# qitianwu/SGFormer

Hardware: AMD Instinct MI355X
Metric: SGFormer fwd+bwd nodes/sec on ogbn-products full-graph (higher is better)
Workload: dtype bf16

## Files before the change

### include/sgf.h

```cpp
#ifndef SGF_H_
#define SGF_H_

#include <stddef.h>
#include <stdint.h>

#ifdef __cplusplus
extern "C" {
#endif

#define SGF_VERSION 661

#define SGF_F32 0
#define SGF_BF16 1
#define SGF_F32_BF16X3 2

#define SGF_OK 0
#define SGF_E_INVALID (-1)
#define SGF_E_WORKSPACE (-2)
#define SGF_E_HIP (-3)
#define SGF_E_UNSUPPORTED (-4)

int sgf_version(void);
const char* sgf_last_error(void);
int sgf_reload_env(void);

size_t sgf_csr_workspace_bytes(int64_t nnz, int64_t n);
int sgf_csr_build(const int64_t* edge_index, int64_t nnz, int64_t n, int64_t* rowptr,
                  int32_t* colind, float* val, int32_t* deg, void* workspace,
                  size_t workspace_bytes, void* stream);

int sgf_csr_transpose(const int64_t* edge_index, int64_t nnz, int64_t n, const int32_t* deg,
                      const int64_t* rowptr, const int32_t* colind, int64_t* t_rowptr,
                      int32_t* t_colind, float* t_val, int32_t* is_symmetric, void* workspace,
                      size_t workspace_bytes, void* stream);

size_t sgf_subgraph_workspace_bytes(int64_t nnz, int64_t n);
int sgf_subgraph_plan(const int64_t* edge_index, int64_t nnz, int64_t n, const int64_t* subset,
                      int64_t m, int32_t* relabel, int64_t* total, void* workspace,
                      size_t workspace_bytes, void* stream);
int sgf_subgraph_emit(const int64_t* edge_index, int64_t nnz, int64_t n, const int32_t* relabel,
                      int32_t relabel_nodes, int64_t total, int64_t* out, int64_t* out_eid,
                      void* workspace, size_t workspace_bytes, void* stream);

size_t sgf_subgraph_csr_plan_workspace_bytes(int64_t m);
size_t sgf_subgraph_csr_emit_workspace_bytes(int64_t m, int64_t total);
int sgf_subgraph_csr_plan(const int64_t* rowptr, const int32_t* colind, int64_t n, const int64_t* subset, int64_t m,
                          int32_t* local_of, int64_t* rowptr_b, int32_t* deg_b, int64_t* total, void* workspace,
                          size_t workspace_bytes, void* stream);
int sgf_subgraph_csr_emit(const int64_t* rowptr, const int32_t* colind, int64_t n, const int64_t* subset, int64_t m,
                          int32_t* local_of, const int64_t* rowptr_b, const int32_t* deg_b, int64_t total, int32_t* colind_b,
                          float* val_b, int64_t* edge_index_b, void* workspace, size_t workspace_bytes, void* stream);

size_t sgf_graph_prologue_workspace_bytes(int64_t m, int64_t n);
int sgf_graph_prologue_plan(const int64_t* edge_index, int64_t m, int64_t n, int32_t to_undirected,
                            int32_t remove_self_loops, int32_t add_self_loops, int64_t* total,
                            void* workspace, size_t workspace_bytes, void* stream);
int sgf_graph_prologue_emit(int64_t m, int64_t n, int32_t to_undirected, int32_t add_self_loops,
                            int64_t total, int64_t* out, void* workspace, size_t workspace_bytes,
                            void* stream);

int sgf_spmm(const int64_t* rowptr, const int32_t* colind, const float* val, const void* x,
             int64_t ldx, int64_t n_cols, void* y, int64_t ldy, int64_t n_rows, int32_t d,
             int32_t dtype, void* stream);

int32_t sgf_spmm_segment_len(void);
size_t sgf_spmm_split_workspace_bytes(int64_t long_segments, int32_t d);
int sgf_spmm_split(const int64_t* rowptr, const int32_t* colind, const float* val, const void* x,
                   int64_t ldx, int64_t n_cols, void* y, int64_t ldy, int64_t n_rows, int32_t d, int32_t dtype,
                   int64_t long_len, int64_t long_segments, void* workspace, size_t workspace_bytes,
                   void* stream);

int sgf_spmm_stream(const int64_t* rowptr, const int32_t* colind, const float* val, const void* x,
                    int64_t ldx, int64_t n_cols, void* y, int64_t ldy, int64_t n_rows, int32_t d, int32_t dtype,
                    int64_t long_len, int64_t long_segments, void* workspace, size_t workspace_bytes,
                    void* stream);

size_t sgf_reorder_workspace_bytes(int64_t nnz, int64_t n);
int sgf_reorder(const int64_t* edge_index, int64_t nnz, int64_t n, int32_t iters1, int32_t iters2,
                int32_t* perm, int32_t* inv, int32_t* community, void* workspace, size_t workspace_bytes,
                void* stream);
size_t sgf_spmm_plan_workspace_bytes(int64_t nnz, int64_t n, int32_t rows_per_block);
int sgf_spmm_plan(const int64_t* rowptr, const int32_t* colind, const float* val, int64_t n, int64_t nnz,
                  int32_t rows_per_block, int32_t lds_rows, int64_t long_len, int32_t* ecode, float* eval,
                  int32_t* nlds, int32_t* sh_ptr, int32_t* sh_cols, int64_t* stats, void* workspace,
                  size_t workspace_bytes, void* stream);
int32_t sgf_spmm_lds_rows_len(int32_t dtype);
int sgf_spmm_blocked(const int64_t* rowptr, const int32_t* ecode, const float* eval, const int32_t* nlds,
                     const int32_t* sh_ptr, const int32_t* sh_cols, const void* x, int64_t ldx, void* y,
                     int64_t ldy, int64_t n_rows, int32_t d, int32_t dtype, int32_t rows_per_block,
                     int32_t lds_rows, int64_t long_len, int64_t long_segments, void* workspace,
                     size_t workspace_bytes, void* stream);

int sgf_spmm_tile_supported(int32_t d, int32_t dtype);
int sgf_spmm_tile_blocks(const int32_t* comm_sorted, int64_t n, int32_t max_rows, int32_t* blk_row,
                         int64_t blk_cap, int64_t* nb_out, void* stream);
size_t sgf_spmm_tile_plan_workspace_bytes(int64_t nnz, int64_t n, int64_t nb);
int sgf_spmm_tile_plan(const int64_t* rowptr, const int32_t* colind, const float* val, int64_t n, int64_t nnz,
                       const int32_t* blk_row, int64_t nb, int32_t cap, int32_t min_count, int64_t long_len,
                       int32_t* ecode, float* eval, int32_t* nlds, int32_t* sh_ptr, int32_t* sh_cols,
                       int64_t* tile_ptr, int64_t* rem_rowptr, int64_t* stats, void* workspace,
                       size_t workspace_bytes, void* stream);
int sgf_spmm_tile_fill(const int64_t* rowptr, const int32_t* ecode, const float* eval, const int32_t* nlds,
                       int64_t n, int64_t nnz, const int32_t* blk_row, int64_t nb, const int64_t* tile_ptr,
                       int64_t n_frag, const int64_t* rem_rowptr, void* tiles, int32_t* rem_col, float* rem_val,
                       void* stream);
int32_t sgf_spmm_tile_sparse_len(void);
size_t sgf_spmm_tile_pack_workspace_bytes(int64_t n_frag);
int sgf_spmm_tile_pack_layout(const int32_t* blk_row, int64_t nb, const int64_t* tile_ptr, const void* tiles,
                              int64_t n_frag, int32_t* grp, int64_t* pool_units, void* workspace,
                              size_t workspace_bytes, void* stream);
int sgf_spmm_tile_pack(const int32_t* blk_row, int64_t nb, const int64_t* tile_ptr, const void* tiles, int64_t n_frag,
                       const int32_t* grp, void* pool, int64_t pool_units, void* stream);
int sgf_spmm_tile(const int32_t* blk_row, int64_t nb, int32_t block_rows, const int32_t* sh_ptr, const int32_t* sh_cols,
                  const int64_t* tile_ptr, const int32_t* grp, const void* pool, const int64_t* rem_rowptr,
                  const int32_t* rem_col, const float* rem_val, const void* x, int64_t ldx, int64_t n_cols, void* y, int64_t ldy,
                  int64_t n_rows, int32_t d, int32_t dtype, int64_t long_len, int64_t long_segments,
                  void* workspace, size_t workspace_bytes, void* stream);

size_t sgf_neighbor_sample_workspace_bytes(int64_t m, int64_t edge_cap);
int sgf_neighbor_sample_mark(int32_t* local_of, const int32_t* ids, int64_t count, int32_t base, void* stream);
int sgf_neighbor_sample_hop(const int64_t* rowptr, const int32_t* colind, const int32_t* frontier, int64_t m,
                            int32_t frontier_local0, int32_t fanout, uint64_t seed, uint64_t batch, int32_t hop,
                            int32_t* local_of, int32_t n_known, int64_t edge_cap, int32_t* edge_src_local,
                            int32_t* edge_dst_local, int32_t* src_global, int32_t* new_nodes, int64_t* counts,
                            void* workspace, size_t workspace_bytes, void* stream);

size_t sgf_neighbor_sample_batch_workspace_bytes(int64_t batch_size, const int32_t* fanouts, int32_t hops, int64_t* node_cap,
                                                  int64_t* edge_cap);
int sgf_neighbor_sample_batch(const int64_t* rowptr, const int32_t* colind, const int32_t* seeds, int64_t batch_size,
                              const int32_t* fanouts, int32_t hops, uint64_t seed, uint64_t batch, int32_t* local_of,
                              int32_t* nodes, int64_t node_cap, int32_t* edge_src_local, int32_t* edge_dst_local,
                              int64_t edge_cap, int64_t* counts, void* workspace, size_t workspace_bytes, void* stream);

int32_t sgf_sampled_csr_supported(int32_t max_fanout);
size_t sgf_sampled_csr_build_workspace_bytes(int64_t node_cap, int64_t edge_cap);
int sgf_sampled_csr_build(const int32_t* edge_src_local, const int32_t* edge_dst_local, const int64_t* counts,
                          int64_t node_cap, int64_t edge_cap, int32_t max_fanout, int64_t* rowptr_b, int32_t* colind_b,
                          float* val_b, int32_t* deg_b, void* workspace, size_t workspace_bytes, void* stream);
size_t sgf_sampled_csr_transpose_workspace_bytes(int64_t n, int64_t nnz);
int sgf_sampled_csr_transpose(const int64_t* rowptr, const int32_t* colind, const float* val, int64_t n, int64_t nnz,
                              int64_t* t_rowptr, int32_t* t_colind, float* t_val, void* workspace, size_t workspace_bytes,
                              void* stream);

int sgf_gather_rows(const void* src, int64_t lds, int32_t src_dtype, int64_t n_src, const void* idx,
                    int32_t idx_is_int64, int64_t n_out, int32_t d, void* dst, int64_t ldd,
                    int32_t dst_dtype, void* stream);
// ... 17 lines not shown

int64_t sgf_attn_bstats_len(int32_t heads, int32_t d);

int sgf_attn_bwd_reduce(const void* q, int64_t ldq, const void* g, int64_t ldg, const void* o,
                        int64_t ldo, const float* den, int64_t n, int32_t heads, int32_t d,
                        int32_t dtype, float* bstats, void* workspace, size_t workspace_bytes,
                        void* stream);

int sgf_attn_bwd_apply(const void* q, int64_t ldq, const void* k, int64_t ldk, const void* v,
                       int64_t ldv, const void* g, int64_t ldg, const void* o, int64_t ldo,
                       const float* den, int64_t n, double n_total, int32_t heads,
                       int32_t v_heads, int32_t d, int32_t dtype, const float* stats,
                       float* bstats, void* dq, int64_t lddq, void* dk, int64_t lddk,
                       void* dv, int64_t lddv, void* stream);
int sgf_attn_bwd_reduce_heads(const void* q, int64_t ldq, const void* g, int64_t ldg, const void* o, int64_t ldo,
                              const float* den, int64_t n, int32_t heads, int32_t d, int32_t dtype, float* bstats,
                              void* workspace, size_t workspace_bytes, void* stream);
int sgf_attn_bwd_apply_heads(const void* q, int64_t ldq, const void* k, int64_t ldk, const void* v, int64_t ldv, const void* g,
                             int64_t ldg, const void* o, int64_t ldo, const float* den, int64_t n, double n_total,
                             int32_t heads, int32_t v_heads, int32_t d, int32_t dtype, const float* stats, float* bstats,
                             void* dq, int64_t lddq, void* dk, int64_t lddk, void* dv, int64_t lddv, void* stream);

int64_t sgf_attn_h_bstats_len(int32_t d);
int32_t sgf_attn_h_supported(int32_t d, int32_t dtype);
int sgf_attn_h_fwd(const void* h, int64_t ldh, int64_t n, int32_t d, int32_t dtype, const float* M,
                   const float* m, const float* w, const float* beta, void* out, int64_t ldo,
                   float* den, void* stream);
int sgf_attn_h_bwd_reduce(const void* h, int64_t ldh, const void* g, int64_t ldg, const void* o,
                          int64_t ldo, const float* den, int64_t n, int32_t d, int32_t dtype,
                          float* hstats, void* workspace, size_t workspace_bytes, void* stream);
int sgf_attn_h_bwd_apply(const void* h, int64_t ldh, const void* g, int64_t ldg, const void* o,
                         int64_t ldo, const float* den, int64_t n, int32_t d, int32_t dtype,
                         const float* M, const float* w, const float* D, const float* ds, void* dh,
                         int64_t lddh, void* workspace, size_t workspace_bytes, void* stream);
size_t sgf_attn_h_bwd_apply_workspace_bytes(int64_t n, int32_t d, int32_t dtype);
int32_t sgf_attn_h_bwd_split_supported(int32_t d, int32_t dtype);
int sgf_attn_h_bwd_pre(const void* g, int64_t ldg, const void* o, int64_t ldo, const float* den, int64_t n, int32_t d,
                       int32_t dtype, const float* M, const float* w, void* workspace, size_t workspace_bytes,
                       float* rowscal, void* stream);
int sgf_attn_h_bwd_reduce_scaled(const void* h, int64_t ldh, const void* g, int64_t ldg, const float* rowscal, int64_t n,
                                 int32_t d, int32_t dtype, float* hstats, void* workspace, size_t workspace_bytes,
                                 void* stream);
int sgf_attn_h_bwd_post(const void* h, int64_t ldh, int64_t n, int32_t d, int32_t dtype, const float* D, const float* ds,
                        const void* workspace, size_t workspace_bytes, const void* addend, int64_t ldadd, void* dh,
                        int64_t lddh, void* stream);

size_t sgf_attn_h_small_saved_bytes(int32_t d_in, int32_t d_out);
size_t sgf_attn_h_small_workspace_bytes(int32_t d_in, int32_t d_out);
int sgf_attn_h_small_fwd(const float* G, int64_t ldg, const float* s, float n_rows, float n_total, const float* wq,
                         const float* bq, const float* wk, const float* bk, const float* wv, const float* bv, int64_t ldw,
                         int32_t d_in, int32_t d_out, float* M, int64_t ldm, float* m, float* w, float* beta, void* saved,
                         size_t saved_bytes, void* stream);
int sgf_attn_h_small_bwd(const float* dM, int64_t lddm, const float* dw, const float* dm, const float* dbeta, float n_total,
                         int32_t d_in, int32_t d_out, const void* saved, size_t saved_bytes, float* dG2, int64_t lddg,
                         float* ds, float* gwq, float* gbq, float* gwk, float* gbk, float* gwv, float* gbv, int64_t ldgw,
                         void* workspace, size_t workspace_bytes, void* stream);

size_t sgf_gram_workspace_bytes(int64_t n, int32_t m, int32_t k);
int sgf_gram(const void* a, int64_t lda, int32_t m, const void* b, int64_t ldb, int32_t k,
             int64_t n, int32_t dtype, float* c, int64_t ldc, float* colsum_a, void* workspace,
             size_t workspace_bytes, void* stream);
int sgf_gram2(const void* a, int64_t lda, int32_t m, const void* b1, int64_t ldb1, const void* b2, int64_t ldb2, int32_t k,
              int64_t n, int32_t dtype, float* c1, int64_t ldc1, float* c2, int64_t ldc2, float* colsum_a, void* workspace,
              size_t workspace_bytes, void* stream);

int sgf_ln_fwd(const void* x, int64_t ldx, const void* res, int64_t ldr, float a, float b,
               const float* gamma, const float* beta, int32_t relu, float eps, int64_t n,
               int32_t d, int32_t dtype, void* y, int64_t ldy, float* mean, float* rstd,
               void* stream);

size_t sgf_ln_bwd_workspace_bytes(int64_t n, int32_t d);
int sgf_ln_bwd(const void* dy, int64_t lddy, const void* y, int64_t ldy, const void* x,
               int64_t ldx, const void* res, int64_t ldr, float a, float b, const float* gamma,
               int32_t relu, const float* mean, const float* rstd, int64_t n, int32_t d,
               int32_t dtype, void* dx, int64_t lddx, void* dres, int64_t lddres, float* dgamma,
               float* dbeta, void* workspace, size_t workspace_bytes, void* stream);

size_t sgf_colstats_workspace_bytes(int64_t n, int32_t d);
int sgf_colstats(const void* x, int64_t ldx, const float* shift, int64_t n, int32_t d,
                 int32_t dtype, float* stats, void* workspace, size_t workspace_bytes,
                 void* stream);
int sgf_bn_finalize(const float* sums, const float* shift, double n_total, float eps, float momentum, float* running_mean,
                    float* running_var, int32_t d, float* mean, float* rstd, void* stream);
int sgf_bn_apply(const void* x, int64_t ldx, const float* mean, const float* rstd,
                 const float* gamma, const float* beta, const void* res, int64_t ldr,
                 int32_t relu, int64_t n, int32_t d, int32_t dtype, void* y, int64_t ldy,
                 void* stream);
int sgf_bn_bwd_stats(const void* dy, int64_t lddy, const void* x, int64_t ldx, const float* mean,
                     const float* rstd, const float* gamma, const float* beta, int32_t relu,
                     int64_t n, int32_t d, int32_t dtype, float* stats, void* workspace,
                     size_t workspace_bytes, void* stream);
int sgf_bn_bwd_stats2(const void* dy, int64_t lddy, const void* dy2, int64_t lddy2, const void* x, int64_t ldx,
                      const float* mean, const float* rstd, const float* gamma, const float* beta, int32_t relu, int64_t n,
                      int32_t d, int32_t dtype, float* stats, void* workspace, size_t workspace_bytes, void* stream);
int32_t sgf_gram_ln_bwd_supported(int32_t m, int32_t k, int32_t dtype);
int sgf_gram_ln_bwd(const void* g, int64_t ldg, const void* xin, int64_t ldx, const float* mean, const float* rstd,
                    const float* gamma, const float* beta, int32_t relu, int32_t m, const void* b, int64_t ldb, int32_t k,
                    int64_t n, int32_t dtype, float* c, int64_t ldc, float* colsum, float* dgamma, float* dbeta, void* workspace,
                    size_t workspace_bytes, void* stream);
int32_t sgf_gram_bn_bwd_supported(int32_t m, int32_t k, int32_t dtype);
int sgf_gram_bn_bwd(const void* g1, int64_t ldg1, const void* g2, int64_t ldg2, const void* z, int64_t ldz, const float* mean,
                    const float* rstd, const float* gamma, const float* beta, int32_t relu, const float* stats, float inv_n,
                    int32_t training, int32_t m, const void* b, int64_t ldb, int32_t k, int64_t n, int32_t dtype, float* c,
                    int64_t ldc, float* colsum, void* workspace, size_t workspace_bytes, void* stream);
int32_t sgf_gram2_bn_bwd_supported(int32_t m, int32_t k, int64_t n, int32_t dtype);
int sgf_gram2_bn_bwd(const void* g, int64_t ldg, const void* z, int64_t ldz, const float* mean, const float* rstd,
                     const float* gamma, const float* beta, int32_t relu, const float* stats, float inv_n, int32_t training,
                     int32_t m, const void* b1, int64_t ldb1, const void* b2, int64_t ldb2, int32_t k, int64_t n, int32_t dtype,
                     void* dz, int64_t lddz, float* c1, int64_t ldc1, float* c2, int64_t ldc2, float* colsum, void* workspace,
                     size_t workspace_bytes, void* stream);
int sgf_bn_bwd_apply(const void* dy, int64_t lddy, const void* x, int64_t ldx, const float* mean,
                     const float* rstd, const float* gamma, const float* beta, int32_t relu,
                     const float* stats, float inv_n, int32_t training, int64_t n, int32_t d,
                     int32_t dtype, void* dx, int64_t lddx, void* stream);

int32_t sgf_combine_fc_supported(int32_t d, int32_t classes, int32_t dtype);
int sgf_combine_fc_fwd(const void* x1, int64_t ld1, float a, const void* x2, int64_t ld2, float b,
                       const float* w, const float* bias, int64_t n, int32_t d, int32_t classes,
                       int32_t dtype, float* logits, int64_t ldl, void* stream);
int sgf_combine_fc_bwd(const float* dlogits, int64_t lddl, const float* w, int64_t n, int32_t d,
                       int32_t classes, float a, float b, int32_t dtype, void* dx1, int64_t ld1, void* dx2,
                       int64_t ld2, void* stream);
int sgf_combine_fc_fwd_mapped(const void* x1, int64_t ld1, float a, const void* x2, int64_t ld2, float b, const float* w,
                              const float* bias, int64_t n, int32_t d, int32_t classes, int32_t dtype, float* logits,
                              int64_t ldl, const int32_t* row_map, void* stream);
int sgf_combine_fc_bwd_mapped(const float* dlogits, int64_t lddl, const float* w, int64_t n, int32_t d, int32_t classes,
                              float a, float b, int32_t dtype, void* dx1, int64_t ld1, void* dx2, int64_t ld2,
                              const int32_t* row_map, void* stream);
int sgf_combine_fc_bwd_g(const float* dlogits, int64_t lddl, const float* w, int64_t n, int32_t d, int32_t classes, float a,
                         float b, int32_t dtype, void* dx1, int64_t ld1, void* dx2, int64_t ld2, const int32_t* row_map,
                         void* g_out, int64_t ldg, void* stream);

int32_t sgf_gcn_epilogue_supported(int32_t d_in, int32_t d_out, int32_t dtype);
size_t sgf_gcn_epilogue_workspace_bytes(int64_t n, int32_t d_out);
int sgf_gcn_epilogue_stats(const void* a, int64_t lda, const void* w, int64_t ldw, const float* bias,
                           int64_t n, int32_t d_in, int32_t d_out, int32_t dtype, void* y, int64_t ldy,
                           const float* shift, float* stats, void* workspace, size_t workspace_bytes,
                           void* stream);
int sgf_gcn_epilogue_dx2(const void* dy, int64_t lddy, const void* w1, const void* w2, int64_t ldw, int64_t n, int32_t d,
                         int32_t dtype, void* dx1, int64_t lddx1, void* dx2, int64_t lddx2, int32_t pair, void* stream);

int32_t sgf_gcn_epilogue_dx2_acc_supported(int32_t d, int32_t dtype);
int sgf_gcn_epilogue_dx2_acc(const void* dz, int64_t lddz, const void* w, int64_t ldw, int64_t n, int32_t d, int32_t dtype,
                             void* dy, int64_t lddy, const void* gadd, int64_t ldg, const void* acc_in, int64_t ldai,
                             void* acc_out, int64_t ldao, void* stream);
int sgf_gcn_epilogue_dx(const void* dy, int64_t lddy, const void* w, int64_t ldw, int64_t n, int32_t d_in,
                        int32_t d_out, int32_t dtype, void* dx, int64_t lddx, void* stream);
int sgf_gcn_epilogue_apply(const void* y, int64_t ldy, const float* mean, const float* rstd, const float* gamma,
                           const float* beta, const void* res, int64_t ldr, int32_t relu, int64_t n, int32_t d,
                           int32_t dtype, void* out, int64_t ldo, void* stream);
int32_t sgf_gcn_bn_bwd_dx_supported(int32_t d, int32_t dtype);
size_t sgf_gcn_bn_bwd_dx_workspace_bytes(int64_t n, int32_t d);
int sgf_gcn_bn_bwd_dx(const void* gy, int64_t ldg, const void* z, int64_t ldz, const float* mean, const float* rstd,
                      const float* gamma, const float* beta, int32_t relu, const float* stats, float inv_n,
                      int32_t training, const void* w, int64_t ldw, int64_t n, int32_t d, int32_t dtype, void* dz,
                      int64_t lddz, void* dy, int64_t lddy, const void* acc_in, void* acc_out, size_t acc_bytes,
                      void* dx0, int64_t lddx0, int32_t add_gy, void* workspace, size_t workspace_bytes, void* stream);
int32_t sgf_gcn_epilogue_cat_supported(int32_t d, int32_t dtype);
int sgf_gcn_epilogue_cat(const void* a1, int64_t lda1, const void* a2, int64_t lda2, const void* w, int64_t ldw,
                         const float* bias, int64_t n, int32_t d, int32_t dtype, void* y, int64_t ldy, const float* shift,
                         float* stats, void* workspace, size_t workspace_bytes, void* stream);
size_t sgf_gcn_epilogue_partial_bytes(int64_t n, int32_t d_out);
size_t sgf_gcn_epilogue_dtype_partial_bytes(int64_t n, int32_t d_out, int32_t dtype);
int sgf_gcn_epilogue_partial(const void* a, int64_t lda, const void* w, int64_t ldw, const float* bias, int64_t n,
                             int32_t d_in, int32_t d_out, int32_t dtype, void* partial, size_t partial_bytes,
                             void* stream);
// ... 78 lines not shown
```

### sgformer_amd/_lib.py

```python
from __future__ import annotations

import ctypes
import os
from ctypes import c_char_p, c_double, c_float, c_int32, c_int64, c_size_t, c_uint64, c_void_p

_HERE = os.path.dirname(os.path.abspath(__file__))
LIB_PATH = os.path.join(_HERE, "lib", "libsgf.so")

SGF_F32 = 0
SGF_BF16 = 1
SGF_F32_BF16X3 = 2
SGF_BCE_TARGET_F32 = 0
SGF_BCE_TARGET_I64 = 1
SGF_BCE_TARGET_CLASS = 2
SGF_METRIC_TARGET_F32 = 0
SGF_METRIC_TARGET_I64 = 1

_lib = None

_P = c_void_p
SIGNATURES = {
    "sgf_version": (c_int32, []),
    "sgf_last_error": (c_char_p, []),
    "sgf_reload_env": (c_int32, []),
    "sgf_csr_workspace_bytes": (c_size_t, [c_int64, c_int64]),
    "sgf_csr_build": (c_int32, [_P, c_int64, c_int64, _P, _P, _P, _P, _P, c_size_t, _P]),
    "sgf_csr_transpose": (c_int32, [_P, c_int64, c_int64, _P, _P, _P, _P, _P, _P, _P, _P, c_size_t, _P]),
    "sgf_subgraph_workspace_bytes": (c_size_t, [c_int64, c_int64]),
    "sgf_subgraph_plan": (c_int32, [_P, c_int64, c_int64, _P, c_int64, _P, _P, _P, c_size_t, _P]),
    "sgf_subgraph_emit": (c_int32, [_P, c_int64, c_int64, _P, c_int32, c_int64, _P, _P, _P, c_size_t, _P]),
    "sgf_subgraph_csr_plan_workspace_bytes": (c_size_t, [c_int64]),
    "sgf_subgraph_csr_emit_workspace_bytes": (c_size_t, [c_int64, c_int64]),
    "sgf_subgraph_csr_plan": (c_int32, [_P, _P, c_int64, _P, c_int64, _P, _P, _P, _P, _P, c_size_t, _P]),
    "sgf_subgraph_csr_emit": (c_int32, [_P, _P, c_int64, _P, c_int64, _P, _P, _P, c_int64, _P, _P, _P, _P, c_size_t, _P]),
    "sgf_graph_prologue_workspace_bytes": (c_size_t, [c_int64, c_int64]),
    "sgf_graph_prologue_plan": (c_int32, [_P, c_int64, c_int64, c_int32, c_int32, c_int32, _P, _P, c_size_t, _P]),
    "sgf_graph_prologue_emit": (c_int32, [c_int64, c_int64, c_int32, c_int32, c_int64, _P, _P, c_size_t, _P]),
    "sgf_spmm": (c_int32, [_P, _P, _P, _P, c_int64, c_int64, _P, c_int64, c_int64, c_int32, c_int32, _P]),
    "sgf_spmm_segment_len": (c_int32, []),
    "sgf_spmm_split_workspace_bytes": (c_size_t, [c_int64, c_int32]),
    "sgf_spmm_split": (c_int32, [_P, _P, _P, _P, c_int64, c_int64, _P, c_int64, c_int64, c_int32, c_int32, c_int64,
                                 c_int64, _P, c_size_t, _P]),
    "sgf_spmm_stream": (c_int32, [_P, _P, _P, _P, c_int64, c_int64, _P, c_int64, c_int64, c_int32, c_int32, c_int64,
                                  c_int64, _P, c_size_t, _P]),
    "sgf_reorder_workspace_bytes": (c_size_t, [c_int64, c_int64]),
    "sgf_reorder": (c_int32, [_P, c_int64, c_int64, c_int32, c_int32, _P, _P, _P, _P, c_size_t, _P]),
    "sgf_spmm_plan_workspace_bytes": (c_size_t, [c_int64, c_int64, c_int32]),
    "sgf_spmm_plan": (c_int32, [_P, _P, _P, c_int64, c_int64, c_int32, c_int32, c_int64, _P, _P, _P, _P, _P, _P,
                                _P, c_size_t, _P]),
    "sgf_spmm_lds_rows_len": (c_int32, [c_int32]),
    "sgf_spmm_blocked": (c_int32, [_P, _P, _P, _P, _P, _P, _P, c_int64, _P, c_int64, c_int64, c_int32, c_int32,
                                   c_int32, c_int32, c_int64, c_int64, _P, c_size_t, _P]),
    "sgf_spmm_tile_supported": (c_int32, [c_int32, c_int32]),
    "sgf_spmm_tile_blocks": (c_int32, [_P, c_int64, c_int32, _P, c_int64, _P, _P]),
    "sgf_spmm_tile_plan_workspace_bytes": (c_size_t, [c_int64, c_int64, c_int64]),
    "sgf_spmm_tile_plan": (c_int32, [_P, _P, _P, c_int64, c_int64, _P, c_int64, c_int32, c_int32, c_int64, _P, _P, _P,
                                     _P, _P, _P, _P, _P, _P, c_size_t, _P]),
    "sgf_spmm_tile_fill": (c_int32, [_P, _P, _P, _P, c_int64, c_int64, _P, c_int64, _P, c_int64, _P, _P, _P, _P, _P]),
    "sgf_spmm_tile_sparse_len": (c_int32, []),
    "sgf_spmm_tile_pack_workspace_bytes": (c_size_t, [c_int64]),
    "sgf_spmm_tile_pack_layout": (c_int32, [_P, c_int64, _P, _P, c_int64, _P, _P, _P, c_size_t, _P]),
    "sgf_spmm_tile_pack": (c_int32, [_P, c_int64, _P, _P, c_int64, _P, _P, c_int64, _P]),
    "sgf_spmm_tile": (c_int32, [_P, c_int64, c_int32, _P, _P, _P, _P, _P, _P, _P, _P, _P, c_int64, c_int64, _P, c_int64,
                                c_int64, c_int32, c_int32, c_int64, c_int64, _P, c_size_t, _P]),
    "sgf_neighbor_sample_workspace_bytes": (c_size_t, [c_int64, c_int64]),
    "sgf_neighbor_sample_mark": (c_int32, [_P, _P, c_int64, c_int32, _P]),
    "sgf_neighbor_sample_batch_workspace_bytes": (c_size_t, [c_int64, _P, c_int32, _P, _P]),
    "sgf_neighbor_sample_batch": (c_int32, [_P, _P, _P, c_int64, _P, c_int32, c_uint64, c_uint64, _P, _P, c_int64, _P, _P,
                                            c_int64, _P, _P, c_size_t, _P]),
    "sgf_neighbor_sample_hop": (c_int32, [_P, _P, _P, c_int64, c_int32, c_int32, c_uint64, c_uint64, c_int32, _P, c_int32,
                                          c_int64, _P, _P, _P, _P, _P, _P, c_size_t, _P]),
    "sgf_sampled_csr_supported": (c_int32, [c_int32]),
    "sgf_sampled_csr_build_workspace_bytes": (c_size_t, [c_int64, c_int64]),
    "sgf_sampled_csr_build": (c_int32, [_P, _P, _P, c_int64, c_int64, c_int32, _P, _P, _P, _P, _P, c_size_t, _P]),
    "sgf_sampled_csr_transpose_workspace_bytes": (c_size_t, [c_int64, c_int64]),
    "sgf_sampled_csr_transpose": (c_int32, [_P, _P, _P, c_int64, c_int64, _P, _P, _P, _P, c_size_t, _P]),
    "sgf_gather_rows": (c_int32, [_P, c_int64, c_int32, c_int64, _P, c_int32, c_int64, c_int32, _P, c_int64,
                                  c_int32, _P]),
    "sgf_pad_rows": (c_int32, [_P, c_int64, c_int32, c_int64, _P, c_int32, c_int64, c_int32, c_int32, _P, c_int64,
                               c_int32, _P]),
    "sgf_attn_stats_len": (c_int64, [c_int32, c_int32]),
    "sgf_attn_bstats_len": (c_int64, [c_int32, c_int32]),
    "sgf_attn_workspace_bytes": (c_size_t, [c_int64, c_int32, c_int32]),
    "sgf_attn_max_blocks": (c_int32, []),
    "sgf_attn_tile_rows": (c_int32, [c_int32, c_int32, c_int32]),
    "sgf_attn_fwd_reduce": (c_int32, [_P, c_int64, _P, c_int64, _P, c_int64, c_int64, c_int32, c_int32,
                                      c_int32, c_int32, _P, _P, c_size_t, _P]),
    "sgf_attn_fwd_apply": (c_int32, [_P, c_int64, _P, c_int64, c_int64, c_double, c_int32, c_int32,
                                     c_int32, c_int32, _P, _P, c_int64, _P, _P, _P]),
    "sgf_attn_bwd_reduce": (c_int32, [_P, c_int64, _P, c_int64, _P, c_int64, _P, c_int64, c_int32,
                                      c_int32, c_int32, _P, _P, c_size_t, _P]),
    "sgf_attn_bwd_apply": (c_int32, [_P, c_int64, _P, c_int64, _P, c_int64, _P, c_int64, _P, c_int64,
                                     _P, c_int64, c_double, c_int32, c_int32, c_int32, c_int32, _P, _P,
                                     _P, c_int64, _P, c_int64, _P, c_int64, _P]),
    "sgf_attn_bwd_reduce_heads": (c_int32, [_P, c_int64, _P, c_int64, _P, c_int64, _P, c_int64, c_int32,
                                            c_int32, c_int32, _P, _P, c_size_t, _P]),
    "sgf_attn_bwd_apply_heads": (c_int32, [_P, c_int64, _P, c_int64, _P, c_int64, _P, c_int64, _P, c_int64,
                                           _P, c_int64, c_double, c_int32, c_int32, c_int32, c_int32, _P, _P,
                                           _P, c_int64, _P, c_int64, _P, c_int64, _P]),
    "sgf_attn_h_bstats_len": (c_int64, [c_int32]),
    "sgf_attn_h_fwd": (c_int32, [_P, c_int64, c_int64, c_int32, c_int32, _P, _P, _P, _P, _P, c_int64, _P, _P]),
    "sgf_attn_h_bwd_reduce": (c_int32, [_P, c_int64, _P, c_int64, _P, c_int64, _P, c_int64, c_int32, c_int32,
                                        _P, _P, c_size_t, _P]),
    "sgf_attn_h_bwd_apply": (c_int32, [_P, c_int64, _P, c_int64, _P, c_int64, _P, c_int64, c_int32, c_int32,
                                       _P, _P, _P, _P, _P, c_int64, _P, c_size_t, _P]),
    "sgf_attn_h_bwd_apply_workspace_bytes": (c_size_t, [c_int64, c_int32, c_int32]),
    "sgf_attn_h_bwd_split_supported": (c_int32, [c_int32, c_int32]),
    "sgf_attn_h_supported": (c_int32, [c_int32, c_int32]),
    "sgf_attn_h_bwd_pre": (c_int32, [_P, c_int64, _P, c_int64, _P, c_int64, c_int32, c_int32, _P, _P, _P, c_size_t, _P, _P]),
    "sgf_attn_h_bwd_reduce_scaled": (c_int32, [_P, c_int64, _P, c_int64, _P, c_int64, c_int32, c_int32, _P, _P, c_size_t,
                                               _P]),
    "sgf_attn_h_bwd_post": (c_int32, [_P, c_int64, c_int64, c_int32, c_int32, _P, _P, _P, c_size_t, _P, c_int64, _P,
                                      c_int64, _P]),
    "sgf_attn_h_small_saved_bytes": (c_size_t, [c_int32, c_int32]),
    "sgf_attn_h_small_workspace_bytes": (c_size_t, [c_int32, c_int32]),
    "sgf_attn_h_small_fwd": (c_int32, [_P, c_int64, _P, c_float, c_float, _P, _P, _P, _P, _P, _P, c_int64, c_int32, c_int32,
                                       _P, c_int64, _P, _P, _P, _P, c_size_t, _P]),
    "sgf_attn_h_small_bwd": (c_int32, [_P, c_int64, _P, _P, _P, c_float, c_int32, c_int32, _P, c_size_t, _P, c_int64, _P,
                                       _P, _P, _P, _P, _P, _P, c_int64, _P, c_size_t, _P]),
    "sgf_gram_workspace_bytes": (c_size_t, [c_int64, c_int32, c_int32]),
    "sgf_gram": (c_int32, [_P, c_int64, c_int32, _P, c_int64, c_int32, c_int64, c_int32, _P, c_int64, _P,
                           _P, c_size_t, _P]),
    "sgf_gram2": (c_int32, [_P, c_int64, c_int32, _P, c_int64, _P, c_int64, c_int32, c_int64, c_int32, _P, c_int64, _P,
                            c_int64, _P, _P, c_size_t, _P]),
    "sgf_ln_fwd": (c_int32, [_P, c_int64, _P, c_int64, c_float, c_float, _P, _P, c_int32, c_float,
                             c_int64, c_int32, c_int32, _P, c_int64, _P, _P, _P]),
    "sgf_ln_bwd_workspace_bytes": (c_size_t, [c_int64, c_int32]),
    "sgf_ln_bwd": (c_int32, [_P, c_int64, _P, c_int64, _P, c_int64, _P, c_int64, c_float, c_float, _P,
                             c_int32, _P, _P, c_int64, c_int32, c_int32, _P, c_int64, _P, c_int64, _P,
                             _P, _P, c_size_t, _P]),
    "sgf_colstats_workspace_bytes": (c_size_t, [c_int64, c_int32]),
    "sgf_colstats": (c_int32, [_P, c_int64, _P, c_int64, c_int32, c_int32, _P, _P, c_size_t, _P]),
    "sgf_bn_finalize": (c_int32, [_P, _P, c_double, c_float, c_float, _P, _P, c_int32, _P, _P, _P]),
    "sgf_bn_apply": (c_int32, [_P, c_int64, _P, _P, _P, _P, _P, c_int64, c_int32, c_int64, c_int32,
                               c_int32, _P, c_int64, _P]),
    "sgf_bn_bwd_stats": (c_int32, [_P, c_int64, _P, c_int64, _P, _P, _P, _P, c_int32, c_int64, c_int32,
                                   c_int32, _P, _P, c_size_t, _P]),
    "sgf_bn_bwd_stats2": (c_int32, [_P, c_int64, _P, c_int64, _P, c_int64, _P, _P, _P, _P, c_int32, c_int64, c_int32,
                                    c_int32, _P, _P, c_size_t, _P]),
    "sgf_gram_ln_bwd_supported": (c_int32, [c_int32, c_int32, c_int32]),
    "sgf_gram_ln_bwd": (c_int32, [_P, c_int64, _P, c_int64, _P, _P, _P, _P, c_int32, c_int32, _P, c_int64, c_int32, c_int64,
                                  c_int32, _P, c_int64, _P, _P, _P, _P, c_size_t, _P]),
    "sgf_gram_bn_bwd_supported": (c_int32, [c_int32, c_int32, c_int32]),
    "sgf_gram_bn_bwd": (c_int32, [_P, c_int64, _P, c_int64, _P, c_int64, _P, _P, _P, _P, c_int32, _P, c_float, c_int32,
                                  c_int32, _P, c_int64, c_int32, c_int64, c_int32, _P, c_int64, _P, _P, c_size_t, _P]),
    "sgf_gram2_bn_bwd_supported": (c_int32, [c_int32, c_int32, c_int64, c_int32]),
    "sgf_gram2_bn_bwd": (c_int32, [_P, c_int64, _P, c_int64, _P, _P, _P, _P, c_int32, _P, c_float, c_int32, c_int32, _P, c_int64,
                                   _P, c_int64, c_int32, c_int64, c_int32, _P, c_int64, _P, c_int64, _P, c_int64, _P, _P,
                                   c_size_t, _P]),
    "sgf_bn_bwd_apply": (c_int32, [_P, c_int64, _P, c_int64, _P, _P, _P, _P, c_int32, _P, c_float,
                                   c_int32, c_int64, c_int32, c_int32, _P, c_int64, _P]),
    "sgf_dropout": (c_int32, [_P, c_int64, _P, c_int64, c_float, c_uint64, c_int64, c_int32, c_int32, _P,
                              c_int64, _P]),
    "sgf_dropout_dev": (c_int32, [_P, c_int64, _P, c_int64, c_float, _P, c_int64, c_int32, c_int32, _P,
                                  c_int64, _P]),
    "sgf_nll_workspace_bytes": (c_size_t, [c_int64]),
    "sgf_nll_fwd": (c_int32, [_P, c_int64, c_int64, c_int32, c_int32, _P, _P, c_int64, _P, _P, c_size_t, _P]),
    "sgf_nll_bwd": (c_int32, [_P, c_int64, c_int64, c_int32, c_int32, _P, _P, c_int64, _P, c_float, _P,
                              c_int64, _P]),
    "sgf_bce_workspace_bytes": (c_size_t, [c_int64, c_int32]),
    "sgf_bce_fwd": (c_int32, [_P, c_int64, c_int64, c_int32, c_int32, _P, c_int64, c_int32, _P, c_int64, c_float, _P, _P,
                              c_size_t, _P]),
    "sgf_bce_bwd": (c_int32, [_P, c_int64, c_int64, c_int32, c_int32, _P, c_int64, c_int32, _P, c_int64, _P, c_float, _P,
                              c_int64, _P]),
    "sgf_rocauc_workspace_bytes": (c_size_t, [c_int64, c_int32]),
    "sgf_rocauc_counts": (c_int32, [_P, c_int64, c_int64, c_int32, c_int32, _P, c_int64, c_int32, _P, c_int64, _P, _P,
                                    c_size_t, _P]),
    "sgf_argmax_workspace_bytes": (c_size_t, [c_int64, c_int32]),
    "sgf_argmax_count": (c_int32, [_P, c_int64, c_int64, c_int32, c_int32, _P, c_int64, c_int32, _P, c_int64, _P, _P,
                                   c_size_t, _P]),
    "sgf_sum_n": (c_int32, [_P, _P, c_int32, c_int64, c_int32, c_int32, _P, c_int64, _P]),
    "sgf_colsum_workspace_bytes": (c_size_t, [c_int64, c_int32]),
    "sgf_colsum": (c_int32, [_P, c_int64, c_int64, c_int32, c_int32, _P, _P, c_size_t, _P]),
    "sgf_combine_fc_supported": (c_int32, [c_int32, c_int32, c_int32]),
    "sgf_combine_fc_fwd": (c_int32, [_P, c_int64, c_float, _P, c_int64, c_float, _P, _P, c_int64, c_int32, c_int32,
                                     c_int32, _P, c_int64, _P]),
    "sgf_combine_fc_bwd": (c_int32, [_P, c_int64, _P, c_int64, c_int32, c_int32, c_float, c_float, c_int32, _P,
                                     c_int64, _P, c_int64, _P]),
    "sgf_combine_fc_fwd_mapped": (c_int32, [_P, c_int64, c_float, _P, c_int64, c_float, _P, _P, c_int64, c_int32, c_int32,
                                     c_int32, _P, c_int64, _P, _P]),
    "sgf_combine_fc_bwd_g": (c_int32, [_P, c_int64, _P, c_int64, c_int32, c_int32, c_float, c_float, c_int32, _P, c_int64, _P,
                                       c_int64, _P, _P, c_int64, _P]),
    "sgf_combine_fc_bwd_mapped": (c_int32, [_P, c_int64, _P, c_int64, c_int32, c_int32, c_float, c_float, c_int32, _P,
                                     c_int64, _P, c_int64, _P, _P]),
    "sgf_gcn_epilogue_supported": (c_int32, [c_int32, c_int32, c_int32]),
    "sgf_gcn_epilogue_workspace_bytes": (c_size_t, [c_int64, c_int32]),
    "sgf_gcn_epilogue_stats": (c_int32, [_P, c_int64, _P, c_int64, _P, c_int64, c_int32, c_int32, c_int32, _P, c_int64,
                                         _P, _P, _P, c_size_t, _P]),
    "sgf_gcn_epilogue_dx": (c_int32, [_P, c_int64, _P, c_int64, c_int64, c_int32, c_int32, c_int32, _P, c_int64, _P]),
    "sgf_gcn_epilogue_dx2": (c_int32, [_P, c_int64, _P, _P, c_int64, c_int64, c_int32, c_int32, _P, c_int64, _P, c_int64,
                                       c_int32, _P]),
    "sgf_gcn_epilogue_dx2_acc_supported": (c_int32, [c_int32, c_int32]),
    "sgf_gcn_epilogue_dx2_acc": (c_int32, [_P, c_int64, _P, c_int64, c_int64, c_int32, c_int32, _P, c_int64, _P, c_int64, _P,
                                           c_int64, _P, c_int64, _P]),
    "sgf_gcn_epilogue_apply": (c_int32, [_P, c_int64, _P, _P, _P, _P, _P, c_int64, c_int32, c_int64, c_int32,
                               c_int32, _P, c_int64, _P]),
    "sgf_gcn_bn_bwd_dx_supported": (c_int32, [c_int32, c_int32]),
    "sgf_gcn_bn_bwd_dx_workspace_bytes": (c_size_t, [c_int64, c_int32]),
    "sgf_gcn_bn_bwd_dx": (c_int32, [_P, c_int64, _P, c_int64, _P, _P, _P, _P, c_int32, _P, c_float, c_int32, _P, c_int64,
                                    c_int64, c_int32, c_int32, _P, c_int64, _P, c_int64, _P, _P, c_size_t, _P, c_int64,
                                    c_int32, _P, c_size_t, _P]),
    "sgf_gcn_epilogue_cat_supported": (c_int32, [c_int32, c_int32]),
    "sgf_gcn_epilogue_cat": (c_int32, [_P, c_int64, _P, c_int64, _P, c_int64, _P, c_int64, c_int32, c_int32, _P, c_int64,
                                       _P, _P, _P, c_size_t, _P]),
    "sgf_gcn_epilogue_partial_bytes": (c_size_t, [c_int64, c_int32]),
    "sgf_gcn_epilogue_dtype_partial_bytes": (c_size_t, [c_int64, c_int32, c_int32]),
    "sgf_gcn_epilogue_partial": (c_int32, [_P, c_int64, _P, c_int64, _P, c_int64, c_int32, c_int32, c_int32, _P,
                                           c_size_t, _P]),
    "sgf_gcn_epilogue_stats_add": (c_int32, [_P, c_int64, _P, c_int64, _P, c_size_t, c_int64, c_int32, c_int32,
                                             c_int32, _P, c_int64, _P, _P, _P, c_size_t, _P]),
    "sgf_stem_pair_supported": (c_int32, [c_int32, c_int32, c_int32]),
    "sgf_stem_pair": (c_int32, [_P, c_int64, c_int64, c_int32, _P, c_int64, _P, _P, c_int64, _P, c_int32, c_int32, _P,
                                c_int64, _P, c_int64, _P, _P, _P, c_size_t, _P]),
    "sgf_gemm": (c_int32, [_P, c_int64, c_int64, c_int32, _P, c_int64, c_int64, c_int32, c_int64, c_int32, c_int64, c_float,
                           _P, _P, c_float, _P, c_int64, c_int32, _P, c_int64, c_int32, _P]),
    "sgf_comm_available": (c_int32, []),
# ... 49 lines not shown
```

### sgformer_amd/csrc/fused.hip

```cpp
#include "common.h"

namespace sgf {
namespace {

constexpr int kThreads = 256;
constexpr int kMaxD = 1024;
constexpr int kMaxStatBlocks = 2048;

__device__ __forceinline__ float4 zero4() { return make_float4(0.f, 0.f, 0.f, 0.f); }
__device__ __forceinline__ float4 ld4f(const float* p) { return *reinterpret_cast<const float4*>(p); }

inline int lanes_per_row(int d) {
  int l = 16;
  while (l * 4 < d && l < 64) l <<= 1;
  return l;
}

template <typename T, int LPR, int NC>
__global__ __launch_bounds__(kThreads) void k_ln_fwd(
    const T* __restrict__ x, int64_t ldx, const T* __restrict__ res, int64_t ldr, float a, float b,
    const float* __restrict__ gamma, const float* __restrict__ beta, int relu, float eps, int64_t n,
    int d, T* __restrict__ y, int64_t ldy, float* __restrict__ mean, float* __restrict__ rstd) {
  constexpr int RPB = kThreads / LPR;
  const int sl = threadIdx.x % LPR;
// ... 1309 lines not shown

extern "C" size_t sgf_ln_bwd_workspace_bytes(int64_t n, int32_t d) {
  (void)n;
  if (d < 1) return 0;
  return static_cast<size_t>(kMaxStatBlocks) * 2 * d * sizeof(float);
}

extern "C" int sgf_ln_bwd(const void* dy, int64_t lddy, const void* y, int64_t ldy, const void* x,
                          int64_t ldx, const void* res, int64_t ldr, float a, float b,
                          const float* gamma, int32_t relu, const float* mean, const float* rstd,
                          int64_t n, int32_t d, int32_t dtype, void* dx, int64_t lddx, void* dres,
                          int64_t lddres, float* dgamma, float* dbeta, void* workspace,
                          size_t workspace_bytes, void* stream) {
  int rc = check_ew("sgf_ln_bwd", n, d, dtype);
  if (rc != SGF_OK) return rc;
  hipStream_t st = static_cast<hipStream_t>(stream);
  if (n == 0) {
    if (gamma && dgamma) SGF_CHECK_HIP(hipMemsetAsync(dgamma, 0, d * sizeof(float), st));
    if (gamma && dbeta) SGF_CHECK_HIP(hipMemsetAsync(dbeta, 0, d * sizeof(float), st));
    return SGF_OK;
  }
  SGF_REQUIRE(dy && dx && (!relu || y) && (!gamma || (x && mean && rstd)), SGF_E_INVALID,
              "sgf_ln_bwd: null pointer");
  SGF_REQUIRE(!gamma || (workspace && workspace_bytes >= sgf_ln_bwd_workspace_bytes(n, d)),
              SGF_E_WORKSPACE, "sgf_ln_bwd: workspace too small");
  if (dtype == SGF_F32)
    return ln_bwd_t<float>(dy, lddy, y, ldy, x, ldx, res, ldr, a, b, gamma, relu, mean, rstd, n, d,
                           dx, lddx, dres, lddres, dgamma, dbeta, workspace, st);
  return ln_bwd_t<uint16_t>(dy, lddy, y, ldy, x, ldx, res, ldr, a, b, gamma, relu, mean, rstd, n, d,
                            dx, lddx, dres, lddres, dgamma, dbeta, workspace, st);
}

extern "C" size_t sgf_colstats_workspace_bytes(int64_t n, int32_t d) {
  (void)n;
  if (d < 1) return 0;
  return static_cast<size_t>(kMaxStatBlocks) * 2 * d * sizeof(float);
}

extern "C" int sgf_colstats(const void* x, int64_t ldx, const float* shift, int64_t n, int32_t d,
                            int32_t dtype, float* stats, void* workspace, size_t workspace_bytes,
                            void* stream) {
  int rc = check_ew("sgf_colstats", n, d, dtype);
  if (rc != SGF_OK) return rc;
  hipStream_t st = static_cast<hipStream_t>(stream);
  SGF_REQUIRE(stats, SGF_E_INVALID, "sgf_colstats: null stats");
  if (n == 0) {
    SGF_CHECK_HIP(hipMemsetAsync(stats, 0, 2 * d * sizeof(float), st));
    return SGF_OK;
  }
  SGF_REQUIRE(x && ldx % 4 == 0, SGF_E_INVALID, "sgf_colstats: bad x / ldx");
  SGF_REQUIRE(workspace && workspace_bytes >= sgf_colstats_workspace_bytes(n, d), SGF_E_WORKSPACE,
              "sgf_colstats: workspace too small");
  if (dtype == SGF_F32)
    return colreduce(ColStatsF<float>{static_cast<const float*>(x), ldx, shift}, n, d, stats,
                     workspace, st);
  return colreduce(ColStatsF<uint16_t>{static_cast<const uint16_t*>(x), ldx, shift}, n, d, stats,
                   workspace, st);
}

__global__ __launch_bounds__(256) void k_bn_finalize(const float* __restrict__ sums, const float* __restrict__ shift,
                                                     float inv_n, float unbias, float eps, float momentum,
                                                     float* __restrict__ rmean, float* __restrict__ rvar, int d,
                                                     float* __restrict__ mean, float* __restrict__ rstd) {
  const int c = blockIdx.x * 256 + threadIdx.x;
  if (c >= d) return;
  const float m1 = sums[c] * inv_n;
  const float mu = (shift ? shift[c] : 0.f) + m1;
  float var = sums[d + c] * inv_n - m1 * m1;
  var = var > 0.f ? var : 0.f;
  mean[c] = mu;
  rstd[c] = 1.0f / sqrtf(var + eps);
  if (rmean) rmean[c] = rmean[c] * (1.0f - momentum) + momentum * mu;
  if (rvar) rvar[c] = rvar[c] * (1.0f - momentum) + momentum * (var * unbias);
}

extern "C" int sgf_bn_finalize(const float* sums, const float* shift, double n_total, float eps, float momentum,
                               float* running_mean, float* running_var, int32_t d, float* mean, float* rstd, void* stream) {
  SGF_REQUIRE(d >= 1 && n_total >= 0, SGF_E_INVALID, "sgf_bn_finalize: bad sizes");
  SGF_REQUIRE(sums && mean && rstd, SGF_E_INVALID, "sgf_bn_finalize: null pointer");
  const double nn = n_total > 1.0 ? n_total : 1.0;
  const float unbias = static_cast<float>(n_total / (n_total - 1.0 > 1.0 ? n_total - 1.0 : 1.0));
  hipLaunchKernelGGL(k_bn_finalize, dim3((d + 255) / 256), dim3(256), 0, static_cast<hipStream_t>(stream), sums, shift,
                     static_cast<float>(1.0 / nn), unbias, eps, momentum, running_mean, running_var, d, mean, rstd);
  SGF_LAUNCH_CHECK();
  return SGF_OK;
}

extern "C" int sgf_bn_apply(const void* x, int64_t ldx, const float* mean, const float* rstd,
                            const float* gamma, const float* beta, const void* res, int64_t ldr,
                            int32_t relu, int64_t n, int32_t d, int32_t dtype, void* y, int64_t ldy,
                            void* stream) {
  int rc = check_ew("sgf_bn_apply", n, d, dtype);
  if (rc != SGF_OK) return rc;
  if (n == 0) return SGF_OK;
  SGF_REQUIRE(x && y && mean && rstd, SGF_E_INVALID, "sgf_bn_apply: null pointer");
  SGF_REQUIRE(ldx % 4 == 0 && ldy % 4 == 0 && (!res || ldr % 4 == 0), SGF_E_INVALID,
              "sgf_bn_apply: leading dims must be multiples of 4");
  hipStream_t st = static_cast<hipStream_t>(stream);
  const BnParams p{mean, rstd, gamma, beta};
  if (dtype == SGF_BF16 && ew8_rows(d, {{x, ldx}, {res, ldr}, {y, ldy}})) {
    const dim3 g8(rowwalk8_grid(n, d));
#define SGF_BNA(RES_, U_)                                                                                             \
  hipLaunchKernelGGL((k_bn_apply_bf16x8<RES_, U_>), g8, dim3(kThreads), 0, st, static_cast<const uint16_t*>(x), ldx, p, \
                     static_cast<const uint16_t*>(res), ldr, relu, n, d, static_cast<uint16_t*>(y), ldy)
    if (res) SGF_BNA(true, kEw8Unroll);
    else SGF_BNA(false, kEw8Unroll);
#undef SGF_BNA
    SGF_LAUNCH_CHECK();
    return SGF_OK;
  }
  const dim3 grid(rowwalk_grid(n, d));
  if (dtype == SGF_F32)
    hipLaunchKernelGGL((k_bn_apply<float>), grid, dim3(kThreads), 0, st,
                       static_cast<const float*>(x), ldx, p, static_cast<const float*>(res), ldr,
                       relu, n, d, static_cast<float*>(y), ldy);
  else
    hipLaunchKernelGGL((k_bn_apply<uint16_t>), grid, dim3(kThreads), 0, st,
                       static_cast<const uint16_t*>(x), ldx, p, static_cast<const uint16_t*>(res),
                       ldr, relu, n, d, static_cast<uint16_t*>(y), ldy);
  SGF_LAUNCH_CHECK();
  return SGF_OK;
}

extern "C" int sgf_bn_bwd_stats2(const void* dy, int64_t lddy, const void* dy2, int64_t lddy2, const void* x, int64_t ldx,
                                 const float* mean, const float* rstd, const float* gamma, const float* beta,
                                 int32_t relu, int64_t n, int32_t d, int32_t dtype, float* stats, void* workspace,
                                 size_t workspace_bytes, void* stream) {
  int rc = check_ew("sgf_bn_bwd_stats2", n, d, dtype);
  if (rc != SGF_OK) return rc;
  hipStream_t st = static_cast<hipStream_t>(stream);
  SGF_REQUIRE(stats, SGF_E_INVALID, "sgf_bn_bwd_stats2: null stats");
  if (n == 0) {
    SGF_CHECK_HIP(hipMemsetAsync(stats, 0, 2 * d * sizeof(float), st));
    return SGF_OK;
  }
  SGF_REQUIRE(dy && x && mean && rstd && lddy % 4 == 0 && ldx % 4 == 0 && (!dy2 || lddy2 % 4 == 0), SGF_E_INVALID,
              "sgf_bn_bwd_stats2: bad pointer / ld");
  SGF_REQUIRE(workspace && workspace_bytes >= sgf_colstats_workspace_bytes(n, d), SGF_E_WORKSPACE,
              "sgf_bn_bwd_stats2: workspace too small");
  const BnParams p{mean, rstd, gamma, beta};
  if (dtype == SGF_BF16 && ew8_rows(d, {{dy, lddy}, {dy2, lddy2}, {x, ldx}})) {
    const int nblk = stat_blocks(n);
    float* part = static_cast<float*>(workspace);
#define SGF_BNS(TWO_, U_)                                                                                             \
  hipLaunchKernelGGL((k_bn_bwd_stats_bf16x8<TWO_, U_>), dim3(nblk), dim3(kThreads), 0, st, static_cast<const uint16_t*>(dy), \
                     lddy, static_cast<const uint16_t*>(dy2), lddy2, static_cast<const uint16_t*>(x), ldx, p, relu, n, d, part)
    if (dy2) SGF_BNS(true, kEw8Unroll);
    else SGF_BNS(false, kEw8Unroll);
#undef SGF_BNS
    SGF_LAUNCH_CHECK();
    hipLaunchKernelGGL(k_sum_partials, dim3((2 * d + 7) / 8), dim3(256), 0, st, part, nblk, 2 * d, stats, stats + d, d);
    SGF_LAUNCH_CHECK();
    return SGF_OK;
  }
  if (dtype == SGF_F32)
    return colreduce(BnBwdStatsF<float>{static_cast<const float*>(dy), lddy, static_cast<const float*>(x), ldx, p, relu,
                                        static_cast<const float*>(dy2), lddy2},
                     n, d, stats, workspace, st);
  return colreduce(BnBwdStatsF<uint16_t>{static_cast<const uint16_t*>(dy), lddy, static_cast<const uint16_t*>(x), ldx, p,
                                         relu, static_cast<const uint16_t*>(dy2), lddy2},
                   n, d, stats, workspace, st);
}

extern "C" int sgf_bn_bwd_stats(const void* dy, int64_t lddy, const void* x, int64_t ldx,
                                const float* mean, const float* rstd, const float* gamma,
                                const float* beta, int32_t relu, int64_t n, int32_t d,
// ... 332 lines not shown
```

### sgformer_amd/csrc/spmm.hip

```cpp
#include "common.h"
#include "spmm_shared.h"

#include <climits>
#include <cstdlib>

namespace sgf {
namespace {

constexpr int kWavesPerBlock = 4;

__device__ __forceinline__ void fma4(float4& acc, float v, const float4& x) {
  acc.x = fmaf(v, x.x, acc.x);
  acc.y = fmaf(v, x.y, acc.y);
  acc.z = fmaf(v, x.z, acc.z);
  acc.w = fmaf(v, x.w, acc.w);
}

template <typename T, int UNROLL>
__global__ __launch_bounds__(kWavesPerBlock * 64) void k_spmm_wave(
    const int64_t* __restrict__ rowptr, const int32_t* __restrict__ colind,
    const float* __restrict__ val, const T* __restrict__ x, int64_t ldx, T* __restrict__ y,
    int64_t ldy, int64_t n_rows, int32_t d, LongQueue lq) {
  const int lane = threadIdx.x & 63;
  const int wid = __builtin_amdgcn_readfirstlane(static_cast<int>(threadIdx.x >> 6));
  const int64_t blk = xcd_remap(blockIdx.x, gridDim.x);
  const int64_t row = blk * kWavesPerBlock + wid;
  if (row >= n_rows) return;
  const int64_t e0 = rowptr[row];
  const int64_t e1 = rowptr[row + 1];
  if (e1 - e0 > lq.long_len) {
    push_long_row(lq, row, e1 - e0, lane, 64);
    return;
  }

  for (int f0 = 0; f0 < d; f0 += 256) {
    const int fc = f0 + lane * 4;
    const bool active = fc < d;
    const T* xl = x + (active ? fc : 0);
    float4 acc = make_float4(0.f, 0.f, 0.f, 0.f);
    int64_t e = e0;
    for (; e + UNROLL <= e1; e += UNROLL) {
      int32_t c[UNROLL];
      float v[UNROLL];
      float4 xv[UNROLL];
#pragma unroll
      for (int u = 0; u < UNROLL; ++u) {
        c[u] = colind[e + u];
        v[u] = val[e + u];
      }
#pragma unroll
      for (int u = 0; u < UNROLL; ++u)
        xv[u] = load4<T>(xl + static_cast<int64_t>(c[u]) * ldx);
#pragma unroll
      for (int u = 0; u < UNROLL; ++u) fma4(acc, v[u], xv[u]);
    }
    for (; e < e1; ++e) {
      const int32_t c = colind[e];
      const float v = val[e];
      const float4 xv = load4<T>(xl + static_cast<int64_t>(c) * ldx);
      fma4(acc, v, xv);
    }
    if (active) store4<T>(y + row * ldy + fc, acc);
  }
}

template <typename T> struct BufRow;
template <> struct BufRow<uint16_t> {
  using Raw = u32x2;
  static __device__ __forceinline__ Raw load(__amdgpu_buffer_rsrc_t r, int voff, uint32_t soff) {
    return __builtin_amdgcn_raw_buffer_load_b64(r, voff, static_cast<int>(soff), 0);
  }
  static __device__ __forceinline__ float4 widen(const Raw& v) {
    float4 f;
    f.x = __uint_as_float(v.x << 16);
    f.y = __uint_as_float(v.x & 0xffff0000u);
    f.z = __uint_as_float(v.y << 16);
    f.w = __uint_as_float(v.y & 0xffff0000u);
    return f;
  }
};
template <> struct BufRow<float> {
  using Raw = u32x4;
  static __device__ __forceinline__ Raw load(__amdgpu_buffer_rsrc_t r, int voff, uint32_t soff) {
    return __builtin_amdgcn_raw_buffer_load_b128(r, voff, static_cast<int>(soff), 0);
  }
  static __device__ __forceinline__ float4 widen(const Raw& v) {
    return make_float4(__uint_as_float(v.x), __uint_as_float(v.y), __uint_as_float(v.z), __uint_as_float(v.w));
  }
};

template <typename T, int N>
__device__ __forceinline__ void gather_batch(__amdgpu_buffer_rsrc_t rsrc, int voff, uint32_t pitch,
                                             const int32_t* __restrict__ colind, const float* __restrict__ val,
                                             int e, float4& acc) {
  int32_t c[N];
  float v[N];
  typename BufRow<T>::Raw raw[N];
#pragma unroll
  for (int u = 0; u < N; ++u) {
    c[u] = colind[e + u];
    v[u] = val[e + u];
  }
#pragma unroll
  for (int u = 0; u < N; ++u) raw[u] = BufRow<T>::load(rsrc, voff, static_cast<uint32_t>(c[u]) * pitch);
#pragma unroll
  for (int u = 0; u < N; ++u) fma4(acc, v[u], BufRow<T>::widen(raw[u]));
}

template <typename T, int UNROLL>
__global__ __launch_bounds__(kWavesPerBlock * 64) void k_spmm_row(
    const int64_t* __restrict__ rowptr, const int32_t* __restrict__ colind, const float* __restrict__ val,
    const T* __restrict__ x, uint32_t pitch, uint32_t x_bytes, T* __restrict__ y, int64_t ldy, int64_t n_rows,
    int32_t d, LongQueue lq) {
  const int lane = threadIdx.x & 63;
  const int wid = __builtin_amdgcn_readfirstlane(static_cast<int>(threadIdx.x >> 6));
  const int64_t blk = xcd_remap(blockIdx.x, gridDim.x);
  const int64_t row = blk * kWavesPerBlock + wid;
  if (row >= n_rows) return;
  const int64_t e0 = rowptr[row];
  const int64_t e1 = rowptr[row + 1];
  if (e1 - e0 > lq.long_len) {
    push_long_row(lq, row, e1 - e0, lane, 64);
    return;
  }
  const __amdgpu_buffer_rsrc_t rsrc = __builtin_amdgcn_make_buffer_rsrc(const_cast<T*>(x), 0, x_bytes, 0x00020000);
  const int fc = lane * 4;
  const bool active = fc < d;
  const int voff = active ? fc * static_cast<int>(sizeof(T)) : 0;
  float4 acc = make_float4(0.f, 0.f, 0.f, 0.f);
  const int32_t* __restrict__ ci = colind + e0;
  const float* __restrict__ va = val + e0;
  const int len = static_cast<int>(e1 - e0);
  int i = 0;
  if (UNROLL <= len) {
    int32_t c0[UNROLL], c1[UNROLL];
    float v0[UNROLL], v1[UNROLL];
    typename BufRow<T>::Raw raw[UNROLL];
#pragma unroll
    for (int u = 0; u < UNROLL; ++u) {
      c0[u] = ci[u];
      v0[u] = va[u];
    }
    for (;;) {
#pragma unroll
      for (int u = 0; u < UNROLL; ++u) raw[u] = BufRow<T>::load(rsrc, voff, static_cast<uint32_t>(c0[u]) * pitch);
      i += UNROLL;
      const bool more_a = i + UNROLL <= len;
      if (more_a) {
#pragma unroll
        for (int u = 0; u < UNROLL; ++u) {
          c1[u] = ci[i + u];
          v1[u] = va[i + u];
        }
      }
#pragma unroll
      for (int u = 0; u < UNROLL; ++u) fma4(acc, v0[u], BufRow<T>::widen(raw[u]));
      if (!more_a) break;
#pragma unroll
      for (int u = 0; u < UNROLL; ++u) raw[u] = BufRow<T>::load(rsrc, voff, static_cast<uint32_t>(c1[u]) * pitch);
      i += UNROLL;
      const bool more_b = i + UNROLL <= len;
      if (more_b) {
#pragma unroll
        for (int u = 0; u < UNROLL; ++u) {
          c0[u] = ci[i + u];
          v0[u] = va[i + u];
        }
      }
#pragma unroll
      for (int u = 0; u < UNROLL; ++u) fma4(acc, v1[u], BufRow<T>::widen(raw[u]));
      if (!more_b) break;
    }
  }
  if (i + 4 <= len) { gather_batch<T, 4>(rsrc, voff, pitch, ci, va, i, acc); i += 4; }
  if (i + 2 <= len) { gather_batch<T, 2>(rsrc, voff, pitch, ci, va, i, acc); i += 2; }
  if (i < len) gather_batch<T, 1>(rsrc, voff, pitch, ci, va, i, acc);
  if (active) store4<T>(y + row * ldy + fc, acc);
}

constexpr int kSegRows = 4;

template <typename T, int G>
__global__ __launch_bounds__(kWavesPerBlock * 64) void k_spmm_seg(
    const int64_t* __restrict__ rowptr, const int32_t* __restrict__ colind, const float* __restrict__ val,
    const T* __restrict__ x, uint32_t pitch, uint32_t x_bytes, T* __restrict__ y, int64_t ldy, int64_t n_rows,
    int32_t d, int32_t chunk_blocks, LongQueue lq) {
  using Raw = typename BufRow<T>::Raw;
  const int lane = threadIdx.x & 63;
  const int wid = __builtin_amdgcn_readfirstlane(static_cast<int>(threadIdx.x >> 6));
  const int64_t blk = xcd_remap(blockIdx.x, gridDim.x, chunk_blocks);
  const int64_t r_first = (blk * kWavesPerBlock + wid) * kSegRows;
  if (r_first >= n_rows) return;
  const int nr = n_rows - r_first < kSegRows ? static_cast<int>(n_rows - r_first) : kSegRows;
  const __amdgpu_buffer_rsrc_t rsrc = __builtin_amdgcn_make_buffer_rsrc(const_cast<T*>(x), 0, x_bytes, 0x00020000);
  const int fc = lane * 4;
  const bool active = fc < d;
  const int voff = active ? fc * static_cast<int>(sizeof(T)) : 0;
  T* __restrict__ yl = y + r_first * ldy + (active ? fc : 0);

  const int64_t e_first = rowptr[r_first];
  const int64_t end_abs = rowptr[r_first + 1 + (lane < nr ? lane : nr - 1)];
  const int64_t begin_abs = __shfl_up(end_abs, 1, 64);
  const int64_t len_i = end_abs - (lane == 0 ? e_first : begin_abs);
  const bool long_i = lane < nr && len_i > lq.long_len;
  auto lane64 = [&](int64_t v, int i) -> int64_t {
    const uint32_t lo = __builtin_amdgcn_readlane(static_cast<int>(v & 0xffffffff), i);
    const uint32_t hi = __builtin_amdgcn_readlane(static_cast<int>(v >> 32), i);
    return static_cast<int64_t>((static_cast<uint64_t>(hi) << 32) | lo);
  };
  const int64_t total64 = lane64(end_abs, nr - 1) - e_first;
  const int32_t* __restrict__ ci = colind + e_first;
  const float* __restrict__ va = val + e_first;

  if (__ballot(long_i) != 0 || total64 >= (static_cast<int64_t>(1) << 31)) {
    for (int r = 0; r < nr; ++r) {
      const int64_t re = lane64(end_abs, r);
      const int64_t rb = r == 0 ? e_first : lane64(end_abs, r - 1);
      if (re - rb > lq.long_len) {
        push_long_row(lq, r_first + r, re - rb, lane, 64);
        continue;
      }
      float4 acc = make_float4(0.f, 0.f, 0.f, 0.f);
      for (int64_t e = rb; e < re; ++e)
        fma4(acc, val[e], BufRow<T>::widen(BufRow<T>::load(rsrc, voff, static_cast<uint32_t>(colind[e]) * pitch)));
      if (active) store4<T>(yl + r * ldy, acc);
    }
    return;
  }

  const int rel_v = static_cast<int>(end_abs - e_first);
  const int total = static_cast<int>(total64);
  int row = 0;
  int row_end = __builtin_amdgcn_readlane(rel_v, 0);
  float4 acc = make_float4(0.f, 0.f, 0.f, 0.f);
  auto boundary = [&](int p) {
    while (p == row_end && row < nr) {
      if (active) store4<T>(yl + row * ldy, acc);
      acc = make_float4(0.f, 0.f, 0.f, 0.f);
      ++row;
      row_end = row < nr ? __builtin_amdgcn_readlane(rel_v, row < kSegRows ? row : kSegRows - 1) : 0x7fffffff;
    }
  };

  int pos = 0;
  int32_t c0[G], c1[G];
  float v0[G], v1[G];
  Raw raw[G];
  if (G <= total) {
#pragma unroll
    for (int u = 0; u < G; ++u) {
      c0[u] = ci[u];
      v0[u] = va[u];
    }
    for (;;) {
#pragma unroll
      for (int u = 0; u < G; ++u) raw[u] = BufRow<T>::load(rsrc, voff, static_cast<uint32_t>(c0[u]) * pitch);
      const bool more_a = pos + 2 * G <= total;
      if (more_a) {
#pragma unroll
// ... 641 lines not shown
    acc[0] = fmaf(v, __uint_as_float(r.x << 16), acc[0]);
    acc[1] = fmaf(v, __uint_as_float(r.x & 0xffff0000u), acc[1]);
    acc[2] = fmaf(v, __uint_as_float(r.y << 16), acc[2]);
    acc[3] = fmaf(v, __uint_as_float(r.y & 0xffff0000u), acc[3]);
    acc[4] = fmaf(v, __uint_as_float(r.z << 16), acc[4]);
    acc[5] = fmaf(v, __uint_as_float(r.z & 0xffff0000u), acc[5]);
    acc[6] = fmaf(v, __uint_as_float(r.w << 16), acc[6]);
    acc[7] = fmaf(v, __uint_as_float(r.w & 0xffff0000u), acc[7]);
  };
  for (;;) {
    const int ci = it_i;
    const int64_t cp = it_p, ce1 = it_e1;
    uint2* const sc = scratch + buf * kPiece;
    sc[lane] = pre;
    __builtin_amdgcn_fence(__ATOMIC_RELEASE, "wavefront");
    __builtin_amdgcn_wave_barrier();
    __builtin_amdgcn_fence(__ATOMIC_ACQUIRE, "wavefront");
    const bool more = next_piece();
    if (more) pre = fetch(it_p);

    const int64_t e0 = rp(ci);
    const int64_t el = e0 + __builtin_amdgcn_readlane(nl_v, ci);
    const int len = ce1 - cp < kPiece ? static_cast<int>(ce1 - cp) : kPiece;
    const int l1x = el > cp ? (el - cp < len ? static_cast<int>(el - cp) : len) : 0;
    const int d0 = l1x;
    const int l1 = (dbg & 2) ? 0 : l1x;
    if (cp == e0) {
#pragma unroll
      for (int k = 0; k < 8; ++k) acc[k] = 0.f;
    }
    auto get = [&](int i, int b) -> uint2 {
      const int idx = i + hi;
      uint2 c = sc[idx < b ? idx : b - 1];
      if (idx >= b) c.y = 0u;
      return c;
    };

    uint2 cv[DG];
    u32x4 xv[DG];
    const int ng = (dbg & 4) ? 0 : len - d0;
    if (ng > 0) {
#pragma unroll
      for (int u = 0; u < DG; ++u) cv[u] = get(d0 + 2 * u, len);
#pragma unroll
      for (int u = 0; u < DG; ++u) xv[u] = row_load(cv[u].x);
    }
    for (int j = 0; j < l1; j += 2 * LB) {
      uint2 c[LB];
      u32x4 t[LB];
#pragma unroll
      for (int u = 0; u < LB; ++u) c[u] = get(j + 2 * u, l1);
#pragma unroll
      for (int u = 0; u < LB; ++u)
        t[u] = *reinterpret_cast<const u32x4*>(tile + (c[u].x & 0x7fffffffu) * 512 + q * 16);
#pragma unroll
      for (int u = 0; u < LB; ++u) fma8(__uint_as_float(c[u].y), t[u]);
    }
    if (ng > 0) {
#pragma unroll
      for (int u = 0; u < DG; ++u) fma8(__uint_as_float(cv[u].y), xv[u]);
      for (int g = d0 + 2 * DG; g < len; g += 2 * DG) {
#pragma unroll
        for (int u = 0; u < DG; ++u) cv[u] = get(g + 2 * u, len);
#pragma unroll
        for (int u = 0; u < DG; ++u) xv[u] = row_load(cv[u].x);
#pragma unroll
        for (int u = 0; u < DG; ++u) fma8(__uint_as_float(cv[u].y), xv[u]);
      }
    }
    if (cp + kPiece >= ce1) store_row(r_first + ci, acc);
    if (!more) break;
    buf ^= 1;
  }
}

EnvInt g_blk2{"SGF_SPMM_BLK2", 1};
EnvInt g_chunk_rows{"SGF_SPMM_CHUNK_ROWS", 4096};
#ifdef SGF_PROBES
EnvInt g_blk_debug{"SGF_SPMM_BLK_DEBUG", 0};
#endif
enum Forced { kForceNone = -1, kForceWave, kForceRow, kForceSeg, kForceSeg2, kForceSub };
const char* const kForcedWords[] = {"wave", "row", "seg", "seg2", "sub"};
EnvWord g_forced{"SGF_SPMM_KERNEL", kForcedWords, 5};

template <typename T>
int launch_blocked(const int64_t* rowptr, const int32_t* ecode, const float* eval, const int32_t* nlds,
                   const int32_t* sh_ptr, const int32_t* sh_cols, const T* x, int64_t ldx, T* y, int64_t ldy,
                   int64_t n_rows, int32_t d, int32_t rows_per_block, int32_t lds_rows, hipStream_t st,
                   const LongQueue& lq, float* partial) {
  using V = typename Stored<T>::type;
  const int threads = rows_per_block / kBlkRowsPerWave * 64;
  const size_t lds_bytes = static_cast<size_t>(lds_rows) * 64 * sizeof(V) +
                           static_cast<size_t>(threads / 64) * kScratchPerWave;
  const int64_t nb = (n_rows + rows_per_block - 1) / rows_per_block;
  int chunk = 4096 / rows_per_block;
  if (chunk < 1) chunk = 1;
#ifdef SGF_PROBES
  const int dbg = g_blk_debug.get();
#else
  const int dbg = 0;
#endif
  const size_t per_cu = 160 * 1024;
  const bool lean = (per_cu / lds_bytes) * static_cast<size_t>(threads / 64) > 16;
  constexpr int DGd = sizeof(T) == 4 ? 4 : 8, DGl = sizeof(T) == 4 ? 2 : 4;
  auto deep_fn = &k_spmm_blk<T, DGd, DGd, 4>;
  auto lean_fn = &k_spmm_blk<T, DGl, DGl, 8>;
  static thread_local size_t attr_set[4] = {0, 0, 0, 0};
  const int which = (sizeof(T) == 4 ? 0 : 2) + (lean ? 1 : 0);
  if (lds_bytes > attr_set[which]) {
    SGF_CHECK_HIP(hipFuncSetAttribute(lean ? reinterpret_cast<const void*>(lean_fn) : reinterpret_cast<const void*>(deep_fn),
                                      hipFuncAttributeMaxDynamicSharedMemorySize, static_cast<int>(lds_bytes)));
    attr_set[which] = lds_bytes;
  }
  const uint64_t xb = static_cast<uint64_t>(n_rows) * static_cast<uint64_t>(ldx) * sizeof(T);
  if (sizeof(T) == 2 && d % 8 == 0 && d <= 256 && ldx % 8 == 0 && ldy % 8 == 0 && reinterpret_cast<uintptr_t>(x) % 16 == 0 &&
      reinterpret_cast<uintptr_t>(y) % 16 == 0 && xb < (static_cast<uint64_t>(1) << 32) && threads <= 512 &&
      g_blk2.get() != 0) {
    const size_t lds2 = static_cast<size_t>(lds_rows) * 512 + static_cast<size_t>(threads / 64) * kScratchPerWave;
    auto fn2 = &k_spmm_blk2<8, 4>;
    static thread_local size_t attr2 = 0;
    if (lds2 > attr2) {
      SGF_CHECK_HIP(hipFuncSetAttribute(reinterpret_cast<const void*>(fn2), hipFuncAttributeMaxDynamicSharedMemorySize,
                                        static_cast<int>(lds2)));
      attr2 = lds2;
    }
    hipLaunchKernelGGL(fn2, dim3(static_cast<unsigned>(nb)), dim3(threads), lds2, st, rowptr, ecode, eval, nlds, sh_ptr,
                       sh_cols, reinterpret_cast<const uint16_t*>(x), static_cast<uint32_t>(ldx * sizeof(T)),
                       static_cast<uint32_t>(xb), reinterpret_cast<uint16_t*>(y), ldy, n_rows, d, rows_per_block,
                       lds_rows, chunk, lq, dbg);
  } else if (lean)
    hipLaunchKernelGGL(lean_fn, dim3(static_cast<unsigned>(nb)), dim3(threads), lds_bytes, st, rowptr, ecode, eval,
                       nlds, sh_ptr, sh_cols, x, ldx, y, ldy, n_rows, d, rows_per_block, lds_rows, chunk, lq, dbg);
  else
    hipLaunchKernelGGL(deep_fn, dim3(static_cast<unsigned>(nb)), dim3(threads), lds_bytes, st, rowptr, ecode, eval,
                       nlds, sh_ptr, sh_cols, x, ldx, y, ldy, n_rows, d, rows_per_block, lds_rows, chunk, lq, dbg);
  SGF_LAUNCH_CHECK();
  return spmm_long_rows(sizeof(T) == 2 ? SGF_BF16 : SGF_F32, rowptr, ecode, eval, x, ldx, d, lq, partial, y, ldy, st);
}

enum class Arm { SegBf16x2, Seg, Row, Wave, Sub };
struct Choice { Arm arm; int lanes_per_row; };
Choice choose_kernel(int32_t d, size_t elem_size, bool fits32, bool pair_ok, bool stream, int forced) {
  const bool pairs = fits32 && elem_size == 2 && pair_ok;
  const bool narrow_stream = d > 64 && d <= 128 && pairs && forced != kForceSub;
  if (d > 128 || narrow_stream) {
    if (pairs && (stream || forced == kForceSeg2 || (narrow_stream && forced == kForceNone))) return {Arm::SegBf16x2, 0};
    if (fits32 && forced == kForceSeg) return {Arm::Seg, 0};
    if (fits32 && forced != kForceWave) return {Arm::Row, 0};
    return {Arm::Wave, 0};
  }
  return {Arm::Sub, d > 64 ? 32 : d > 32 ? 16 : d > 16 ? 8 : d > 8 ? 4 : d > 4 ? 2 : 1};
}

template <typename T>
int launch(const int64_t* rowptr, const int32_t* colind, const float* val, const T* x, int64_t ldx, int64_t n_cols,
           T* y, int64_t ldy, int64_t n_rows, int32_t d, hipStream_t st, const LongQueue& lq,
           float* partial, bool stream) {
  constexpr int UNROLL = 8;
  const dim3 block(kWavesPerBlock * 64);
  const uint64_t x_bytes = static_cast<uint64_t>(n_cols) * static_cast<uint64_t>(ldx) * sizeof(T);
  const bool fits32 = d <= 256 && n_cols > 0 && x_bytes < (static_cast<uint64_t>(1) << 32);
  const bool pair_ok = d % 8 == 0 && ldx % 8 == 0 && ldy % 8 == 0 && reinterpret_cast<uintptr_t>(x) % 16 == 0 &&
                       reinterpret_cast<uintptr_t>(y) % 16 == 0;
  const Choice c = choose_kernel(d, sizeof(T), fits32, pair_ok, stream, g_forced.get());
  const int64_t nb = (n_rows + kWavesPerBlock - 1) / kWavesPerBlock;
  const int64_t nbs = (n_rows + kWavesPerBlock * kSegRows - 1) / (kWavesPerBlock * kSegRows);
  const int chunk_rows = g_chunk_rows.get() > 0 ? g_chunk_rows.get() : 4096;
  const int chunk = chunk_rows / (kWavesPerBlock * kSegRows) > 0 ? chunk_rows / (kWavesPerBlock * kSegRows) : 1;
#define SGF_SUB(LPR_)                                                                         \
  case LPR_: {                                                                                \
    constexpr int RPB = kWavesPerBlock * (64 / LPR_);                                         \
    const int64_t nbr = (n_rows + RPB - 1) / RPB;                                             \
    hipLaunchKernelGGL((k_spmm_sub<T, LPR_, UNROLL>), dim3(static_cast<unsigned>(nbr)), block, \
                       0, st, rowptr, colind, val, x, ldx, y, ldy, n_rows, d, lq);            \
  } break;
  switch (c.arm) {
    case Arm::SegBf16x2:
      hipLaunchKernelGGL((k_spmm_seg_bf16x2<16>), dim3(static_cast<unsigned>(nbs)), block, 0, st, rowptr, colind, val,
                         reinterpret_cast<const uint16_t*>(x), static_cast<uint32_t>(ldx * sizeof(T)),
                         static_cast<uint32_t>(x_bytes), reinterpret_cast<uint16_t*>(y), ldy, n_rows, d, chunk, lq);
      break;
    case Arm::Seg:
      hipLaunchKernelGGL((k_spmm_seg<T, (sizeof(T) == 4 ? 8 : 16)>), dim3(static_cast<unsigned>(nbs)), block, 0, st,
                         rowptr, colind, val, x, static_cast<uint32_t>(ldx * sizeof(T)),
                         static_cast<uint32_t>(x_bytes), y, ldy, n_rows, d, chunk, lq);
      break;
    case Arm::Row:
      hipLaunchKernelGGL((k_spmm_row<T, UNROLL>), dim3(static_cast<unsigned>(nb)), block, 0, st, rowptr, colind,
                         val, x, static_cast<uint32_t>(ldx * sizeof(T)), static_cast<uint32_t>(x_bytes), y, ldy,
                         n_rows, d, lq);
      break;
    case Arm::Wave:
      hipLaunchKernelGGL((k_spmm_wave<T, UNROLL>), dim3(static_cast<unsigned>(nb)), block, 0, st,
                         rowptr, colind, val, x, ldx, y, ldy, n_rows, d, lq);
      break;
    case Arm::Sub:
      switch (c.lanes_per_row) {
        SGF_SUB(32)
        SGF_SUB(16)
        SGF_SUB(8)
        SGF_SUB(4)
        SGF_SUB(2)
        SGF_SUB(1)
      }
      break;
  }
#undef SGF_SUB
  SGF_LAUNCH_CHECK();
  return spmm_long_rows(sizeof(T) == 2 ? SGF_BF16 : SGF_F32, rowptr, colind, val, x, ldx, d, lq, partial, y, ldy, st);
}

}

int spmm_long_rows(int dtype, const int64_t* rowptr, const int32_t* colind, const float* val, const void* x, int64_t ldx,
                   int32_t d, const LongQueue& lq, float* partial, void* y, int64_t ldy, hipStream_t st) {
  if (lq.cap <= 0) return SGF_OK;
  constexpr int UNROLL = 8;
  const dim3 block(kWavesPerBlock * 64);
  const int nb = lq.cap < 2048 ? lq.cap : 2048;
  if (dtype == SGF_BF16) {
    hipLaunchKernelGGL((k_spmm_long_seg<uint16_t, UNROLL>), dim3(nb), block, 0, st, rowptr, colind, val,
                       static_cast<const uint16_t*>(x), ldx, d, lq, partial);
    SGF_LAUNCH_CHECK();
    hipLaunchKernelGGL((k_spmm_long_fin<uint16_t>), dim3(nb), dim3(256), 0, st, lq, partial, d,
                       static_cast<uint16_t*>(y), ldy);
  } else {
    hipLaunchKernelGGL((k_spmm_long_seg<float, UNROLL>), dim3(nb), block, 0, st, rowptr, colind, val,
                       static_cast<const float*>(x), ldx, d, lq, partial);
    SGF_LAUNCH_CHECK();
    hipLaunchKernelGGL((k_spmm_long_fin<float>), dim3(nb), dim3(256), 0, st, lq, partial, d, static_cast<float*>(y), ldy);
  }
  SGF_LAUNCH_CHECK();
  return SGF_OK;
}

}

using namespace sgf;

namespace {
int check_spmm_operands(const char* fn, const void* x, int64_t ldx, const void* y, int64_t ldy, int32_t d, int32_t dtype) {
  SGF_REQUIRE(dtype == SGF_F32 || dtype == SGF_BF16, SGF_E_INVALID, "%s: unknown dtype %d", fn, dtype);
  SGF_REQUIRE(d % 4 == 0 && ldx % 4 == 0 && ldy % 4 == 0 && ldx >= d && ldy >= d, SGF_E_INVALID,
              "%s: d, ldx, ldy must be multiples of 4 with ld >= d (d=%d ldx=%lld ldy=%lld)", fn, d,
              static_cast<long long>(ldx), static_cast<long long>(ldy));
  const size_t esz = dtype == SGF_BF16 ? 2 : 4;
  SGF_REQUIRE(reinterpret_cast<uintptr_t>(x) % (4 * esz) == 0 && reinterpret_cast<uintptr_t>(y) % (4 * esz) == 0,
              SGF_E_INVALID, "%s: x / y must be aligned to 4 elements", fn);
  return SGF_OK;
}

int spmm_common(const int64_t* rowptr, const int32_t* colind, const float* val, const void* x, int64_t ldx,
                int64_t n_cols, void* y, int64_t ldy, int64_t n_rows, int32_t d, int32_t dtype, const LongQueue& lq,
                float* partial, hipStream_t st, const char* fn, bool stream = false) {
  SGF_REQUIRE(n_rows >= 0 && d >= 0 && n_cols >= 0, SGF_E_INVALID, "%s: negative size", fn);
  if (n_rows == 0 || d == 0) return SGF_OK;
  SGF_REQUIRE(rowptr && x && y, SGF_E_INVALID, "%s: null pointer", fn);
  SGF_REQUIRE(n_rows < (static_cast<int64_t>(1) << 31) * kWavesPerBlock, SGF_E_UNSUPPORTED,
              "%s: n_rows too large for one launch", fn);
  if (const int rc = check_spmm_operands(fn, x, ldx, y, ldy, d, dtype)) return rc;
  if (dtype == SGF_F32)
    return launch<float>(rowptr, colind, val, static_cast<const float*>(x), ldx, n_cols, static_cast<float*>(y), ldy,
                         n_rows, d, st, lq, partial, stream);
  return launch<uint16_t>(rowptr, colind, val, static_cast<const uint16_t*>(x), ldx, n_cols,
                          static_cast<uint16_t*>(y), ldy, n_rows, d, st, lq, partial, stream);
}
}

extern "C" int sgf_spmm(const int64_t* rowptr, const int32_t* colind, const float* val,
                        const void* x, int64_t ldx, int64_t n_cols, void* y, int64_t ldy, int64_t n_rows,
                        int32_t d, int32_t dtype, void* stream) {
  const LongQueue none{nullptr, nullptr, 0, INT64_MAX};
  return spmm_common(rowptr, colind, val, x, ldx, n_cols, y, ldy, n_rows, d, dtype, none, nullptr,
                     static_cast<hipStream_t>(stream), "sgf_spmm");
}

extern "C" int32_t sgf_spmm_segment_len(void) { return kSegLen; }

extern "C" size_t sgf_spmm_split_workspace_bytes(int64_t long_segments, int32_t d) {
  if (long_segments < 0 || d < 0) return 0;
  return long_partial_off(long_segments) + static_cast<size_t>(long_segments) * static_cast<size_t>(d) * sizeof(float);
}

int sgf::spmm_long_queue(const char* fn, int64_t long_len, int64_t long_segments, int32_t d, void* workspace,
                         size_t workspace_bytes, hipStream_t st, LongQueue* lq, float** partial) {
  SGF_REQUIRE(long_len >= 1 && long_segments >= 0 && long_segments < (static_cast<int64_t>(1) << 31),
              SGF_E_INVALID, "%s: bad long_len / long_segments", fn);
  *lq = LongQueue{nullptr, nullptr, 0, INT64_MAX};
  *partial = nullptr;
  if (long_segments == 0) return SGF_OK;
  SGF_REQUIRE(workspace && workspace_bytes >= sgf_spmm_split_workspace_bytes(long_segments, d),
              SGF_E_WORKSPACE, "%s: workspace too small", fn);
  char* ws = static_cast<char*>(workspace);
  lq->count = reinterpret_cast<int32_t*>(ws + kLongCountOff);
  lq->entries = reinterpret_cast<LongEntry*>(ws + kLongEntriesOff);
  lq->cap = static_cast<int32_t>(long_segments);
  lq->long_len = long_len;
  *partial = reinterpret_cast<float*>(ws + long_partial_off(long_segments));
  SGF_CHECK_HIP(hipMemsetAsync(lq->count, 0, sizeof(int32_t), st));
  return SGF_OK;
}

static int spmm_split_impl(bool stream_hint, const char* fn, const int64_t* rowptr, const int32_t* colind, const float* val,
                              const void* x, int64_t ldx, int64_t n_cols, void* y, int64_t ldy, int64_t n_rows,
                              int32_t d, int32_t dtype, int64_t long_len, int64_t long_segments,
                              void* workspace, size_t workspace_bytes, void* stream) {
  hipStream_t st = static_cast<hipStream_t>(stream);
  LongQueue lq;
  float* partial;
  if (const int rc = spmm_long_queue(fn, long_len, long_segments, d, workspace, workspace_bytes, st, &lq, &partial)) return rc;
  return spmm_common(rowptr, colind, val, x, ldx, n_cols, y, ldy, n_rows, d, dtype, lq, partial, st, fn, stream_hint);
}

extern "C" int sgf_spmm_split(const int64_t* rowptr, const int32_t* colind, const float* val, const void* x,
                              int64_t ldx, int64_t n_cols, void* y, int64_t ldy, int64_t n_rows, int32_t d,
                              int32_t dtype, int64_t long_len, int64_t long_segments, void* workspace,
                              size_t workspace_bytes, void* stream) {
  return spmm_split_impl(false, "sgf_spmm_split", rowptr, colind, val, x, ldx, n_cols, y, ldy, n_rows, d, dtype,
                         long_len, long_segments, workspace, workspace_bytes, stream);
}

extern "C" int sgf_spmm_stream(const int64_t* rowptr, const int32_t* colind, const float* val, const void* x,
                               int64_t ldx, int64_t n_cols, void* y, int64_t ldy, int64_t n_rows, int32_t d,
                               int32_t dtype, int64_t long_len, int64_t long_segments, void* workspace,
                               size_t workspace_bytes, void* stream) {
  return spmm_split_impl(true, "sgf_spmm_stream", rowptr, colind, val, x, ldx, n_cols, y, ldy, n_rows, d, dtype,
                         long_len, long_segments, workspace, workspace_bytes, stream);
}

extern "C" int32_t sgf_spmm_lds_rows_len(int32_t dtype) {
  return dtype == SGF_BF16 ? 288 : 144;
}

extern "C" int sgf_spmm_blocked(const int64_t* rowptr, const int32_t* ecode, const float* eval,
                                const int32_t* nlds, const int32_t* sh_ptr, const int32_t* sh_cols,
                                const void* x, int64_t ldx, void* y, int64_t ldy, int64_t n_rows, int32_t d,
                                int32_t dtype, int32_t rows_per_block, int32_t lds_rows, int64_t long_len,
                                int64_t long_segments, void* workspace, size_t workspace_bytes, void* stream) {
  const char* fn = "sgf_spmm_blocked";
  SGF_REQUIRE(n_rows >= 0 && d >= 0, SGF_E_INVALID, "%s: negative size", fn);
  if (n_rows == 0 || d == 0) return SGF_OK;
  SGF_REQUIRE(rowptr && ecode && eval && nlds && sh_ptr && sh_cols && x && y, SGF_E_INVALID, "%s: null pointer", fn);
  SGF_REQUIRE(d <= 256, SGF_E_UNSUPPORTED, "%s: d = %d > 256 (one wave per row)", fn, d);
  SGF_REQUIRE(rows_per_block >= kBlkRowsPerWave && rows_per_block <= 128 && rows_per_block % kBlkRowsPerWave == 0,
              SGF_E_INVALID, "%s: rows_per_block must be a multiple of %d in [%d, 128]", fn, kBlkRowsPerWave,
              kBlkRowsPerWave);
  SGF_REQUIRE(lds_rows >= 1 && lds_rows <= sgf_spmm_lds_rows_len(dtype), SGF_E_INVALID,
              "%s: lds_rows %d outside [1, %d]", fn, lds_rows, sgf_spmm_lds_rows_len(dtype));
  if (const int rc = check_spmm_operands(fn, x, ldx, y, ldy, d, dtype)) return rc;
  hipStream_t st = static_cast<hipStream_t>(stream);
  LongQueue lq;
  float* partial;
  if (const int rc = spmm_long_queue(fn, long_len, long_segments, d, workspace, workspace_bytes, st, &lq, &partial)) return rc;
  if (dtype == SGF_F32)
    return launch_blocked<float>(rowptr, ecode, eval, nlds, sh_ptr, sh_cols, static_cast<const float*>(x), ldx,
                                 static_cast<float*>(y), ldy, n_rows, d, rows_per_block, lds_rows, st, lq, partial);
  return launch_blocked<uint16_t>(rowptr, ecode, eval, nlds, sh_ptr, sh_cols, static_cast<const uint16_t*>(x), ldx,
// ... 3 lines not shown
```

### sgformer_amd/graph.py

```python
from __future__ import annotations

import ctypes
from collections import OrderedDict
from typing import Optional

import torch

from . import _lib
from .kernels import (HipKernels, LONG_ROW, _SEGMENT, _code, _ld, _one_pass_cat, _pair_gram, _ptr, _rows,
                      _rows16, _stream, _workspace, _workspaces)

_F32 = torch.float32
_BF16 = torch.bfloat16


K = HipKernels()



SMALL_GRAPH_NNZ = 1 << 23


def long_row_segments(rowptr: torch.Tensor, nnz: Optional[int] = None, max_row_len: Optional[int] = None) -> int:
    if rowptr.numel() <= 1:
        return 0
    if max_row_len is not None and max_row_len <= LONG_ROW:
        return 0
    if nnz is not None and nnz < SMALL_GRAPH_NNZ:
        return 0 if nnz <= LONG_ROW else nnz // _SEGMENT + nnz // (LONG_ROW + 1) + 1
    lens = rowptr[1:] - rowptr[:-1]
    segs = torch.where(lens > LONG_ROW, (lens + (_SEGMENT - 1)) // _SEGMENT, torch.zeros_like(lens))
    return int(segs.sum())


class CSRGraph:

    def __init__(self, edge_index: torch.Tensor, num_nodes: int, validate: bool = True):
        K.check(edge_index)
        if edge_index.dtype != torch.int64 or edge_index.dim() != 2 or edge_index.shape[0] != 2:
            raise ValueError("edge_index must be an int64 tensor of shape [2, nnz]")
        if num_nodes >= 2 ** 31:
            raise ValueError("num_nodes must be < 2^31 (int32 column indices)")
        ei = edge_index.contiguous()
        n = int(num_nodes)
        if getattr(edge_index, "_sgf_trusted", False):
            validate = False
        if validate and ei.shape[1] > 0:
            lo, hi = torch.aminmax(ei)
            if int(lo) < 0 or int(hi) >= n:
                raise IndexError(f"edge_index has node ids outside [0, {n})")
        self.n, self.nnz, self.device = n, int(ei.shape[1]), ei.device
        self.edge_index = ei
        pre = getattr(edge_index, "_sgf_csr", None)
        if pre is not None and pre[0].numel() == n + 1 and pre[1].numel() == self.nnz:
            self.rowptr, self.colind, self.val, self.deg = pre
            self._t_lazy = bool(getattr(edge_index, "_sgf_csr_t_lazy", False))
        else:
            self.rowptr, self.colind, self.val, self.deg = K.csr_build(ei, n)
        hint = getattr(edge_index, "_sgf_max_in_degree", None)
        self.long_segments = long_row_segments(self.rowptr, self.nnz, None if hint is None else int(hint))
        self.t_long_segments = 0
        self._t = None
        self.symmetric: Optional[bool] = None
        if getattr(edge_index, "_sgf_symmetric", False):
            self.symmetric, self._t, self.t_long_segments = True, (self.rowptr, self.colind, self.val), self.long_segments

    def transposed(self):
        if self._t is None and self._t_lazy:
            self._t = K.sampled_csr_transpose(self.rowptr, self.colind, self.val, self.n)
            self.symmetric = False
            self.t_long_segments = long_row_segments(self._t[0], self.nnz)
        if self._t is None:
            t_rowptr, t_colind, t_val, sym = K.csr_transpose(self.edge_index, self.n, self.deg,
                                                             self.rowptr, self.colind)
            self.symmetric = sym
            self._t = (self.rowptr, self.colind, self.val) if sym else (t_rowptr, t_colind, t_val)
            self.t_long_segments = self.long_segments if sym else long_row_segments(t_rowptr, self.nnz)
        return self._t

    blocked = False
    _t_lazy = False

    def plan(self, dtype, transposed: bool = False):
        if not self.blocked:
            return None
        if not hasattr(self, "_plans"):
            self._plans = {}
        if transposed:
            self.transposed()
            if self.symmetric:
                transposed = False
        key = (bool(transposed), dtype)
        if key not in self._plans:
            rp, ci, va = self.transposed() if transposed else (self.rowptr, self.colind, self.val)
            self._plans[key] = BlockedPlan(rp, ci, va, self.n, dtype)
        return self._plans[key]

    tiled = False
    blk_row = None

    def tile_plan(self, transposed: bool = False):
        if not hasattr(self, "_tile_plans"):
            self._tile_plans = {}
        if transposed:
            self.transposed()
            if self.symmetric:
                transposed = False
        if transposed not in self._tile_plans:
            rp, ci, va = self.transposed() if transposed else (self.rowptr, self.colind, self.val)
            self._tile_plans[transposed] = TilePlan(rp, ci, va, self.n, self.blk_row,
                                                   min_count=getattr(self, "tile_min_count", None))
        return self._tile_plans[transposed]

    def view(self, now: bool = False) -> "GraphView":
        self.forward_calls = getattr(self, "forward_calls", 0) + 1
        v = getattr(self, "_view", None)
        if v is None:
            v = GraphView.decide(self, now)
            if v is not None:
                self._view = v
        return v if v is not None else GraphView(self, None, None)


class WeightedCSRGraph:

    blocked = False

    def __init__(self, edge_index: torch.Tensor, values: torch.Tensor, num_nodes: int):
        K.check(edge_index, values)
        n = int(num_nodes)
        self.n, self.nnz, self.device = n, int(edge_index.shape[1]), edge_index.device
        self._src, self._tgt = edge_index[0].contiguous(), edge_index[1].contiguous()
        self._values = values.detach().to(_F32).contiguous()
        self.rowptr, self.colind, self.val = self._sorted(self._tgt, self._src)
        self.long_segments = long_row_segments(self.rowptr, self.nnz)
        self._t, self.t_long_segments, self.symmetric = None, 0, False

    def _sorted(self, rows, cols):
        perm = torch.argsort(rows * self.n + cols, stable=True)
        counts = torch.bincount(rows, minlength=self.n)
        rowptr = torch.zeros(self.n + 1, dtype=torch.int64, device=self.device)
        torch.cumsum(counts, 0, out=rowptr[1:])
        return rowptr, cols[perm].to(torch.int32), self._values[perm]

    def transposed(self):
        if self._t is None:
            self._t = self._sorted(self._src, self._tgt)
            self.t_long_segments = long_row_segments(self._t[0], self.nnz)
        return self._t

    def plan(self, dtype, transposed=False):
        return None


def weighted_graph(edge_index: torch.Tensor, edge_weight: torch.Tensor, num_nodes: int, value_fn, tag: str):
    key_tag = (tag, edge_weight.data_ptr(), edge_weight._version, tuple(edge_weight.shape))

    def build(ei, n):
        ei2, vals = value_fn(ei, edge_weight, n)
        g = WeightedCSRGraph(ei2, vals, n)
        g.edge_weight_ref = edge_weight
# ... 164 lines not shown
        if getattr(shard, "overlap", False):
            shard.overlapped_exchanges = getattr(shard, "overlapped_exchanges", 0) + 1
            own, (rp_h, ci_h, va_h, seg_h) = plan.split(rowptr, val, n_local)
            recv, work, keep = shard.halo_exchange_start(x, plan)
            y = _own_block_spmm(graph, plan, own, x, n_local, transposed)
            work.wait()
            y.add_(K.spmm(rp_h, ci_h, va_h, recv, n_local, long_segments=seg_h))
            del keep
            return y
        return K.spmm(rowptr, plan.colind, val, shard.halo_exchange(x, plan), n_local, long_segments=long_segments)
    d = x.shape[1]
    chunks = shard.gather_chunks(d)
    if chunks <= 1:
        return K.spmm(rowptr, colind, val, shard.all_gather_rows(x), n_local, long_segments=long_segments)
    w = d // chunks
    pending = [shard.all_gather_rows(x[:, c * w:(c + 1) * w].contiguous(), async_op=True) for c in range(chunks)]
    y = torch.empty((n_local, d), dtype=x.dtype, device=x.device)
    for c, (buf, work) in enumerate(pending):
        work.wait()
        K.spmm(rowptr, colind, val, buf, n_local, out=y[:, c * w:(c + 1) * w], long_segments=long_segments)
    return y


def _own_block_spmm(graph, plan, own, x, n_local: int, transposed: bool):
    rp, ci, va, segs = own
    if getattr(graph, "locality", False):
        import os
        if (hasattr(K, "tile_supported") and K.tile_supported(x.shape[1], x.dtype) and getattr(graph, "comm_local", None) is not None
                and os.environ.get("SGF_SPMM_TILED", "1") == "1" and n_local >= 256
                and x.shape[0] * max(x.stride(0), x.shape[1]) * 2 < 2 ** 32 - 2048):
            plans = plan.__dict__.setdefault("_own_tile_plans", {})
            tp = plans.get("plan")
            if tp is None:
                try:
                    _, _, max_rows = _tile_params()
                    blk_row = K.tile_blocks(graph.comm_local, n_local, max_rows, x.device)
                    tp = TilePlan(rp, ci, va, n_local, blk_row)
                    if tp.tile_fraction < REORDER_MIN_LDS_FRACTION:
                        tp = False
                except (ValueError, _lib.SgfError):
                    tp = False
                plans["plan"] = tp
            if tp:
                return K.spmm_tile(tp, x, n_local)
        return K.spmm(rp, ci, va, x, n_local, long_segments=segs, stream_hint=True)
    return K.spmm(rp, ci, va, x, n_local, long_segments=segs)


class _SpMM(torch.autograd.Function):
    @staticmethod
    def forward(ctx, x, graph, shard):
        K.check(x)
        ctx.graph, ctx.shard = graph, shard
        if shard is not None:
            return _sharded_spmm(graph, x, shard, False)
        return spmm_on(graph, x, False)

    @staticmethod
    def backward(ctx, gy):
        graph, shard = ctx.graph, ctx.shard
        if shard is not None:
            return _sharded_spmm(graph, gy.contiguous(), shard, True), None, None
        return spmm_on(graph, gy.contiguous(), True), None, None


def spmm_on(graph, x: torch.Tensor, transposed: bool, out=None) -> torch.Tensor:
    rp, ci, va = graph.transposed() if transposed else (graph.rowptr, graph.colind, graph.val)
    segs = graph.t_long_segments if transposed else graph.long_segments
    plan = graph.plan(x.dtype, transposed) if (getattr(graph, "blocked", False) and x.shape[1] <= 256) else None
    if plan is not None:
        return K.spmm_blocked(rp, plan, x, graph.n, out=out, long_segments=segs)
    if getattr(graph, "tiled", False):
        if (K.tile_supported(x.shape[1], x.dtype)
                and x.shape[0] * max(x.stride(0), x.shape[1]) * 2 < 2 ** 32 - 2048
                and (out is None or (out.stride(0) % 8 == 0 and out.data_ptr() % 16 == 0))):
            return K.spmm_tile(graph.tile_plan(transposed), x, graph.n, out=out)
        if not K.tile_supported(x.shape[1], x.dtype) and getattr(graph, "_tile_plans", None):
            graph._tile_plans.clear()
    if getattr(graph, "locality", False):
        return K.spmm(rp, ci, va, x, graph.n, out=out, long_segments=segs, stream_hint=True)
    return K.spmm(rp, ci, va, x, graph.n, out=out, long_segments=segs)


def spmm(graph, x: torch.Tensor, shard=None) -> torch.Tensor:
    return _SpMM.apply(x, graph, shard)
```

### sgformer_amd/graphed.py

```python
from __future__ import annotations

import gc
import os
import weakref
from collections import OrderedDict

import torch
import torch.nn as nn

from . import ops

_F32 = torch.float32


_graveyard = []


def collect():
    if _graveyard and not torch.cuda.is_current_stream_capturing():
        torch.cuda.synchronize()
        _graveyard.clear()
        gc.collect()


class _PerModel(OrderedDict):

    def __deepcopy__(self, memo):
        return _PerModel()

    def __del__(self):
        try:
            for e in self.values():
                e.release()
        except Exception:
            pass

    def __reduce__(self):
        return (_PerModel, ())


_MIN_NODES = 4096
_SEEN_BEFORE_CAPTURE = 1
_MAX_CAPTURED = 4
_SEED_RING = 4
counters = {"captures": 0, "replays": 0}


def enabled() -> bool:
    return os.environ.get("SGF_BATCH_GRAPH", "1") != "0" and ops.K.name == "hip" and torch.cuda.is_available()


GRAPH_DROPOUT_DEFAULT = "0"


def graph_dropout() -> bool:
    return os.environ.get("SGF_GRAPH_DROPOUT", GRAPH_DROPOUT_DEFAULT) != "0"


def draw_seeds(k: int, out=None) -> torch.Tensor:
    if out is None:
        out = torch.empty(k, dtype=torch.int64)
    for j in range(k):
        torch.randint(0, 2 ** 62, (1,), dtype=torch.int64, out=out[j:j + 1])
    return out[:k]


def _drop_state(model):
    return tuple(getattr(b, "dropout", None) for b in (model.trans_conv, model.graph_conv))


def _fused_dropout_sites(branch) -> bool:
    fcs = getattr(branch, "fcs", None)
    return fcs is not None and len(fcs) > 0 and fcs[0].out_features % 4 == 0


class StaticCSR(ops.CSRGraph):

    def __init__(self, n: int, cap: int, device, long_segments: int):
        self.n, self.nnz, self.cap, self.device = n, 0, cap, device
        self.edge_index = None
        self.rowptr = torch.zeros(n + 1, dtype=torch.int64, device=device)
        self.colind = torch.zeros(cap, dtype=torch.int32, device=device)
        self.val = torch.zeros(cap, dtype=_F32, device=device)
        self.deg = None
        self.long_segments = self.t_long_segments = int(long_segments)
        self.symmetric = True
        self._t = (self.rowptr, self.colind, self.val)

    def load(self, rowptr, colind, val):
        nnz = self.nnz = int(colind.numel())
        self.rowptr.copy_(rowptr)
        self.colind[:nnz].copy_(colind)
        self.val[:nnz].copy_(val)

    def view(self, now: bool = False):
        return ops.GraphView(self, None, None)


class _Core(nn.Module):

    def __init__(self, model, graph, cdt, out_dtype):
        super().__init__()
        self.model, self.cdt, self.out_dtype = model, cdt, out_dtype
        self._graph = graph

    def forward(self, x):
        m = self.model
        return m._core(m._entry_copy_uncached(x, self.cdt), self._graph, None, None, self.out_dtype)


class _Entry:
    def __init__(self):
        self.seen = 0
        self.core = None
        self.graph = None
        self.params = ()
        self.param_ptrs = None
        self.failed = False
        self.scratch = None
        self.bank = None
        self.drop = None
        self.ring = None
        self.turn = 0
        self.pending = None

    def busy(self) -> bool:
        return self.pending is not None and self.pending() is not None

    def refill(self):
        k = self.bank.used if self.bank is not None else 0
        if k == 0:
            return
        if self.ring is None:
            self.ring = [(torch.empty(self.bank.seeds.numel(), dtype=torch.int64).pin_memory(), torch.cuda.Event())
                         for _ in range(_SEED_RING)]
        self.turn = (self.turn + 1) % _SEED_RING
        host, copied = self.ring[self.turn]
        copied.synchronize()
        draw_seeds(k, host)
        self.bank.seeds[:k].copy_(host[:k], non_blocking=True)
        copied.record()

    def release(self):
        if self.core is not None:
            _graveyard.append((self.core, self.graph, self.scratch, self.bank, self.ring))
        self.core = self.graph = self.pending = self.scratch = self.bank = self.ring = self.drop = None
        self.params, self.param_ptrs = (), None


def _eligible(model, x, edge_index) -> bool:
    if not (enabled() and model.training and torch.is_grad_enabled() and x.is_cuda and not x.requires_grad):
        return False
    if not getattr(edge_index, "_sgf_symmetric", False) or x.shape[0] < _MIN_NODES:
        return False
    csr = edge_index._sgf_csr
    if csr[0].numel() != x.shape[0] + 1 or csr[1].numel() != edge_index.shape[1]:
        return False
    if not model.use_graph or model.graph_conv._shard is not None:
        return False
    for branch in (model.trans_conv, model.graph_conv):
        p = getattr(branch, "dropout", 1.0)
        if p is not None and p > 0.0:
            if not (graph_dropout() and hasattr(branch, "dropout") and hasattr(ops.K, "dropout_dev")
                    and _fused_dropout_sites(branch)):
                return False
    return True


def _long_bound(edge_index, cap: int) -> int:
    hint = getattr(edge_index, "_sgf_max_in_degree", None)
# ... 105 lines not shown
```

### sgformer_amd/kernels.py

```python
from __future__ import annotations

import ctypes
from typing import Optional

import torch

from . import _lib

_F32 = torch.float32
_BF16 = torch.bfloat16

LONG_ROW = 1024
_SEGMENT = 1024


def _ptr(t: Optional[torch.Tensor]):
    return None if t is None else ctypes.c_void_p(t.data_ptr())


def _stream(device) -> ctypes.c_void_p:
    return ctypes.c_void_p(torch.cuda.current_stream(device).cuda_stream)


def _code(t: torch.Tensor) -> int:
# ... 198 lines not shown
                t = 0 if bad else int(t)
                colind_b = torch.empty(t, dtype=torch.int32, device=dev)
                val_b = torch.empty(t, dtype=_F32, device=dev)
                ei_b = torch.empty((2, t), dtype=torch.int64, device=dev) if want_edges else None
                ws2 = _workspace(dev, "subgraph_csr_emit", lib.sgf_subgraph_csr_emit_workspace_bytes(m, t))
            except BaseException:
                local_of.fill_(-1)
                raise
            _lib.call("sgf_subgraph_csr_emit", _ptr(rowptr), _ptr(colind), n, _ptr(subset), m, _ptr(local_of), _ptr(rowptr_b),
                      _ptr(deg_b), t, _ptr(colind_b), _ptr(val_b), _ptr(ei_b), _ptr(ws2), ws2.numel(), _stream(dev))
        if bad:
            return None
        return rowptr_b, colind_b, val_b, deg_b[:m], ei_b, int(longest)

    @staticmethod
    def sampled_csr_supported(max_fanout: int) -> bool:
        return bool(_lib.load().sgf_sampled_csr_supported(int(max_fanout)))

    @staticmethod
    def sampled_csr_build(e_src: torch.Tensor, e_dst: torch.Tensor, counts: torch.Tensor, node_cap: int, edge_cap: int,
                          max_fanout: int):
        dev = e_src.device
        rowptr_b = torch.empty(node_cap + 1, dtype=torch.int64, device=dev)
        colind_b = torch.empty(max(edge_cap, 1), dtype=torch.int32, device=dev)
        val_b = torch.empty(max(edge_cap, 1), dtype=_F32, device=dev)
        deg_b = torch.empty(node_cap + 1, dtype=torch.int32, device=dev)
        ws = _workspace(dev, "sampled_csr_build", _lib.load().sgf_sampled_csr_build_workspace_bytes(node_cap, edge_cap))
        with torch.cuda.device(dev):
            _lib.call("sgf_sampled_csr_build", _ptr(e_src), _ptr(e_dst), _ptr(counts), node_cap, edge_cap, int(max_fanout),
                      _ptr(rowptr_b), _ptr(colind_b), _ptr(val_b), _ptr(deg_b), _ptr(ws), ws.numel(), _stream(dev))
        return rowptr_b, colind_b, val_b, deg_b

    @staticmethod
    def sampled_csr_transpose(rowptr, colind, val, n: int):
        dev, nnz = rowptr.device, int(colind.numel())
        t_rowptr = torch.empty(n + 1, dtype=torch.int64, device=dev)
        t_colind = torch.empty(nnz, dtype=torch.int32, device=dev)
        t_val = torch.empty(nnz, dtype=_F32, device=dev)
        ws = _workspace(dev, "sampled_csr_transpose", _lib.load().sgf_sampled_csr_transpose_workspace_bytes(n, nnz))
        with torch.cuda.device(dev):
            _lib.call("sgf_sampled_csr_transpose", _ptr(rowptr), _ptr(colind), _ptr(val), n, nnz, _ptr(t_rowptr), _ptr(t_colind),
                      _ptr(t_val), _ptr(ws), ws.numel(), _stream(dev))
        return t_rowptr, t_colind, t_val

    @staticmethod
    def graph_prologue(ei: torch.Tensor, n: int, undirected: bool, remove_loops: bool, add_loops: bool):
        dev, m = ei.device, int(ei.shape[1])
        lib = _lib.load()
        total = torch.zeros(1, dtype=torch.int64, device=dev)
        ws = torch.empty(max(lib.sgf_graph_prologue_workspace_bytes(m, n), 256), dtype=torch.uint8, device=dev)
        with torch.cuda.device(dev):
            _lib.call("sgf_graph_prologue_plan", _ptr(ei), m, n, int(undirected), int(remove_loops), int(add_loops),
                      _ptr(total), _ptr(ws), ws.numel(), _stream(dev))
            k = int(total.item())
            out = torch.empty((2, k), dtype=torch.int64, device=dev)
            _lib.call("sgf_graph_prologue_emit", m, n, int(undirected), int(add_loops), k, _ptr(out), _ptr(ws),
                      ws.numel(), _stream(dev))
        return out

    @staticmethod
    def spmm(rowptr, colind, val, x: torch.Tensor, n_rows: int, out: Optional[torch.Tensor] = None,
             long_segments: int = 0, stream_hint: bool = False) -> torch.Tensor:
        x = _rows(x)
        d = x.shape[1]
        y = torch.empty((n_rows, d), dtype=x.dtype, device=x.device) if out is None else out
        if out is not None and (out.shape != (n_rows, d) or out.dtype != x.dtype or out.stride(1) != 1
                                or out.stride(0) % 4 != 0 or out.data_ptr() % (4 * out.element_size()) != 0):
            raise ValueError("spmm: `out` must be [n_rows, d], same dtype, row-contiguous and 4-element aligned")
        if n_rows == 0 or d == 0:
            return y
        with torch.cuda.device(x.device):
            if long_segments > 0 or stream_hint:
                ws = (_workspace(x.device, "spmm_long", _lib.load().sgf_spmm_split_workspace_bytes(long_segments, d))
                      if long_segments > 0 else None)
                _lib.call("sgf_spmm_stream" if stream_hint else "sgf_spmm_split", _ptr(rowptr), _ptr(colind), _ptr(val), _ptr(x), x.stride(0), x.shape[0],
                          _ptr(y), y.stride(0), n_rows, d, _code(x), LONG_ROW, long_segments, _ptr(ws),
                          0 if ws is None else ws.numel(), _stream(x.device))
            else:
                _lib.call("sgf_spmm", _ptr(rowptr), _ptr(colind), _ptr(val), _ptr(x), x.stride(0), x.shape[0],
                          _ptr(y), y.stride(0), n_rows, d, _code(x), _stream(x.device))
        return y

    @staticmethod
    def reorder(ei: torch.Tensor, n: int, iters1: int, iters2: int):
        dev, nnz = ei.device, int(ei.shape[1])
        perm = torch.empty(n, dtype=torch.int32, device=dev)
        inv = torch.empty(n, dtype=torch.int32, device=dev)
        comm = torch.empty(n, dtype=torch.int32, device=dev)
        nbytes = _lib.load().sgf_reorder_workspace_bytes(nnz, n)
        ws = torch.empty(max(nbytes, 256), dtype=torch.uint8, device=dev)
        with torch.cuda.device(dev):
            _lib.call("sgf_reorder", _ptr(ei), nnz, n, int(iters1), int(iters2), _ptr(perm), _ptr(inv),
                      _ptr(comm), _ptr(ws), ws.numel(), _stream(dev))
        return perm, inv, comm

    @staticmethod
    def spmm_plan(rowptr, colind, val, n: int, rows_per_block: int, lds_rows: int, long_len: int):
        dev, nnz = rowptr.device, int(colind.numel())
        nb = (n + rows_per_block - 1) // rows_per_block
        ecode = torch.empty(nnz, dtype=torch.int32, device=dev)
        ev = torch.empty(nnz, dtype=_F32, device=dev)
        nlds = torch.empty(max(n, 1), dtype=torch.int32, device=dev)
        sh_ptr = torch.empty(nb + 1, dtype=torch.int32, device=dev)
        sh_cols = torch.empty(max(nb * lds_rows, 1), dtype=torch.int32, device=dev)
        stats = torch.zeros(4, dtype=torch.int64, device=dev)
        nbytes = _lib.load().sgf_spmm_plan_workspace_bytes(nnz, n, rows_per_block)
        ws = torch.empty(max(nbytes, 256), dtype=torch.uint8, device=dev)
        with torch.cuda.device(dev):
            _lib.call("sgf_spmm_plan", _ptr(rowptr), _ptr(colind), _ptr(val), n, nnz, int(rows_per_block),
                      int(lds_rows), int(long_len), _ptr(ecode), _ptr(ev), _ptr(nlds), _ptr(sh_ptr),
                      _ptr(sh_cols), _ptr(stats), _ptr(ws), ws.numel(), _stream(dev))
        st = [int(v) for v in stats.tolist()]
        return ecode, ev, nlds, sh_ptr, sh_cols[: max(st[1], 1)].clone(), st

    @staticmethod
    def spmm_blocked(rowptr, plan, x: torch.Tensor, n_rows: int, out: Optional[torch.Tensor] = None,
                     long_segments: int = 0) -> torch.Tensor:
        x = _rows(x)
        d = x.shape[1]
        y = torch.empty((n_rows, d), dtype=x.dtype, device=x.device) if out is None else out
        if n_rows == 0 or d == 0:
            return y
        with torch.cuda.device(x.device):
            ws = None
            if long_segments > 0:
                ws = _workspace(x.device, "spmm_long", _lib.load().sgf_spmm_split_workspace_bytes(long_segments, d))
            _lib.call("sgf_spmm_blocked", _ptr(rowptr), _ptr(plan.ecode), _ptr(plan.eval), _ptr(plan.nlds),
                      _ptr(plan.sh_ptr), _ptr(plan.sh_cols), _ptr(x), x.stride(0), _ptr(y), y.stride(0), n_rows, d,
                      _code(x), plan.rows_per_block, plan.lds_rows, LONG_ROW, long_segments, _ptr(ws),
                      0 if ws is None else ws.numel(), _stream(x.device))
        return y

    @staticmethod
    def tile_supported(d: int, dtype) -> bool:
        return bool(_lib.load().sgf_spmm_tile_supported(int(d), _lib.SGF_BF16 if dtype == _BF16 else _lib.SGF_F32))

    @staticmethod
    def tile_blocks(comm_sorted: Optional[torch.Tensor], n: int, max_rows: int, device) -> torch.Tensor:
        cap = 4 * n // int(max_rows) + 4
        blk = torch.empty(cap + 1, dtype=torch.int32, device=device)
        nb = ctypes.c_int64(0)
        with torch.cuda.device(device):
            _lib.call("sgf_spmm_tile_blocks", _ptr(comm_sorted), n, int(max_rows), _ptr(blk), cap, ctypes.byref(nb),
                      _stream(device))
        return blk[: nb.value + 1].clone()

    @staticmethod
    def tile_plan(rowptr, colind, val, n: int, blk_row: torch.Tensor, cap: int, min_count: int, long_len: int):
        dev, nnz, nb = rowptr.device, int(colind.numel()), int(blk_row.numel()) - 1
        ecode = torch.empty(max(nnz, 1), dtype=torch.int32, device=dev)
        ev = torch.empty(max(nnz, 1), dtype=_F32, device=dev)
        nlds = torch.empty(max(n, 1), dtype=torch.int32, device=dev)
        sh_ptr = torch.empty(nb + 1, dtype=torch.int32, device=dev)
        sh_cols = torch.empty(max(nb * cap, 1), dtype=torch.int32, device=dev)
        tile_ptr = torch.empty(nb + 1, dtype=torch.int64, device=dev)
        rem_rowptr = torch.empty(n + 1, dtype=torch.int64, device=dev)
        stats = torch.zeros(8, dtype=torch.int64, device=dev)
        nbytes = _lib.load().sgf_spmm_tile_plan_workspace_bytes(nnz, n, nb)
        ws = torch.empty(max(nbytes, 256), dtype=torch.uint8, device=dev)
        with torch.cuda.device(dev):
            _lib.call("sgf_spmm_tile_plan", _ptr(rowptr), _ptr(colind), _ptr(val), n, nnz, _ptr(blk_row), nb, int(cap),
                      int(min_count), int(long_len), _ptr(ecode), _ptr(ev), _ptr(nlds), _ptr(sh_ptr), _ptr(sh_cols),
                      _ptr(tile_ptr), _ptr(rem_rowptr), _ptr(stats), _ptr(ws), ws.numel(), _stream(dev))
            st = [int(v) for v in stats.tolist()]
            del ws
            if st[7]:
# ... 243 lines not shown
        ws = _workspace(dev, "attn_h_part", _lib.load().sgf_attn_h_bwd_apply_workspace_bytes(n, d, _code(h)))
        dh = torch.empty((n, d), dtype=h.dtype, device=dev)
        with torch.cuda.device(dev):
            _lib.call("sgf_attn_h_bwd_post", _ptr(h), _ld(h), n, d, _code(h), _ptr(D), _ptr(ds), _ptr(ws), ws.numel(),
                      _ptr(addend), 0 if addend is None else _ld(addend), _ptr(dh), dh.stride(0), _stream(dev))
        return dh

    @staticmethod
    def gram(a, b, out=None, want_colsum=True):
        n, m = a.shape
        k = b.shape[1]
        dev = a.device
        if out is None:
            out = torch.empty((m, k), dtype=_F32, device=dev)
        cs = torch.empty(m, dtype=_F32, device=dev) if want_colsum else None
        ws = _workspace(dev, "attn", _lib.load().sgf_gram_workspace_bytes(n, m, k))
        with torch.cuda.device(dev):
            _lib.call("sgf_gram", _ptr(a), _ld(a), m, _ptr(b), _ld(b), k, n, _mm_code(a), _ptr(out),
                      out.stride(0), _ptr(cs), _ptr(ws), ws.numel(), _stream(dev))
        return out, cs

    @staticmethod
    def gram2(a, b1, b2, out1, out2, want_colsum=True):
        n, m = a.shape
        k = b1.shape[1]
        dev = a.device
        cs = torch.empty(m, dtype=_F32, device=dev) if want_colsum else None
        ws = _workspace(dev, "attn", _lib.load().sgf_gram_workspace_bytes(n, m, k))
        with torch.cuda.device(dev):
            _lib.call("sgf_gram2", _ptr(a), _ld(a), m, _ptr(b1), _ld(b1), _ptr(b2), _ld(b2), k, n, _mm_code(a), _ptr(out1),
                      out1.stride(0), _ptr(out2), out2.stride(0), _ptr(cs), _ptr(ws), ws.numel(), _stream(dev))
        return cs

    @staticmethod
    def ln_fwd(x, res, a: float, b: float, gamma, beta, relu: bool, eps: float):
        n, d = x.shape
        dev = x.device
        y = torch.empty((n, d), dtype=x.dtype, device=dev)
        mean = torch.empty(n, dtype=_F32, device=dev) if gamma is not None else None
        rstd = torch.empty(n, dtype=_F32, device=dev) if gamma is not None else None
        with torch.cuda.device(dev):
            _lib.call("sgf_ln_fwd", _ptr(x), _ld(x), _ptr(res), _ld(res), float(a), float(b),
                      _ptr(gamma), _ptr(beta), int(relu), float(eps), n, d, _code(x), _ptr(y),
                      y.stride(0), _ptr(mean), _ptr(rstd), _stream(dev))
        return y, mean, rstd

    @staticmethod
    def ln_bwd(gy, y, x, res, a: float, b: float, gamma, relu: bool, mean, rstd):
        n, d = x.shape
        dev = x.device
        dx = torch.empty_like(x)
        shared = res is not None and float(a) == float(b)
        dres = torch.empty_like(res) if (res is not None and not shared) else None
        dgamma = torch.empty(d, dtype=_F32, device=dev) if gamma is not None else None
        dbeta = torch.empty(d, dtype=_F32, device=dev) if gamma is not None else None
        ws = _workspace(dev, "ln", _lib.load().sgf_ln_bwd_workspace_bytes(n, d))
        with torch.cuda.device(dev):
            _lib.call("sgf_ln_bwd", _ptr(gy), _ld(gy), _ptr(y), _ld(y), _ptr(x), _ld(x), _ptr(res),
                      _ld(res), float(a), float(b), _ptr(gamma), int(relu), _ptr(mean), _ptr(rstd), n,
                      d, _code(x), _ptr(dx), _ld(dx), _ptr(dres), _ld(dres), _ptr(dgamma), _ptr(dbeta),
                      _ptr(ws), ws.numel(), _stream(dev))
        return dx, (dx if shared else dres), dgamma, dbeta

    @staticmethod
    def colstats(x, shift) -> torch.Tensor:
        n, d = x.shape
        dev = x.device
        stats = torch.empty(2 * d, dtype=_F32, device=dev)
        ws = _workspace(dev, "col", _lib.load().sgf_colstats_workspace_bytes(n, d))
        with torch.cuda.device(dev):
            _lib.call("sgf_colstats", _ptr(x), _ld(x), _ptr(shift), n, d, _code(x), _ptr(stats),
                      _ptr(ws), ws.numel(), _stream(dev))
        return stats

    @staticmethod
    def bn_finalize(sums, shift, n_total: float, eps: float, momentum: float, running_mean, running_var):
        d = sums.numel() // 2
        mean = torch.empty(d, dtype=_F32, device=sums.device)
        rstd = torch.empty(d, dtype=_F32, device=sums.device)
        with torch.cuda.device(sums.device):
            _lib.call("sgf_bn_finalize", _ptr(sums), _ptr(shift), float(n_total), float(eps), float(momentum),
                      _ptr(running_mean), _ptr(running_var), d, _ptr(mean), _ptr(rstd), _stream(sums.device))
        return mean, rstd

    @staticmethod
    def bn_apply(x, mean, rstd, gamma, beta, res, relu: bool) -> torch.Tensor:
        n, d = x.shape
        dev = x.device
        y = torch.empty((n, d), dtype=x.dtype, device=dev)
        with torch.cuda.device(dev):
            _lib.call("sgf_bn_apply", _ptr(x), _ld(x), _ptr(mean), _ptr(rstd), _ptr(gamma), _ptr(beta),
                      _ptr(res), _ld(res), int(relu), n, d, _code(x), _ptr(y), y.stride(0),
                      _stream(dev))
        return y

    @staticmethod
    def bn_bwd_stats(gy, x, mean, rstd, gamma, beta, relu: bool) -> torch.Tensor:
        n, d = x.shape
        dev = x.device
        stats = torch.empty(2 * d, dtype=_F32, device=dev)
        ws = _workspace(dev, "col", _lib.load().sgf_colstats_workspace_bytes(n, d))
        with torch.cuda.device(dev):
            _lib.call("sgf_bn_bwd_stats", _ptr(gy), _ld(gy), _ptr(x), _ld(x), _ptr(mean), _ptr(rstd),
                      _ptr(gamma), _ptr(beta), int(relu), n, d, _code(x), _ptr(stats), _ptr(ws),
                      ws.numel(), _stream(dev))
        return stats

    @staticmethod
    def bn_bwd_stats2(gy, gy2, x, mean, rstd, gamma, beta, relu: bool) -> torch.Tensor:
        n, d = x.shape
        dev = x.device
        stats = torch.empty(2 * d, dtype=_F32, device=dev)
        ws = _workspace(dev, "col", _lib.load().sgf_colstats_workspace_bytes(n, d))
        with torch.cuda.device(dev):
            _lib.call("sgf_bn_bwd_stats2", _ptr(gy), _ld(gy), _ptr(gy2), _ld(gy2), _ptr(x), _ld(x), _ptr(mean), _ptr(rstd),
                      _ptr(gamma), _ptr(beta), int(relu), n, d, _code(x), _ptr(stats), _ptr(ws), ws.numel(), _stream(dev))
        return stats

    @staticmethod
    def gram_ln_bwd_supported(m: int, k: int, dtype) -> bool:
        return dtype == _BF16 and bool(_lib.load().sgf_gram_ln_bwd_supported(int(m), int(k), _lib.SGF_BF16))

    @staticmethod
    def gram_ln_bwd(g, xin, mean, rstd, gamma, beta, relu: bool, b):
        n, m = xin.shape
        k = b.shape[1]
        dev = xin.device
        out = torch.empty((m, k), dtype=_F32, device=dev)
        cs = torch.empty(m, dtype=_F32, device=dev)
        dg = torch.empty(m, dtype=_F32, device=dev)
        db = torch.empty(m, dtype=_F32, device=dev)
        ws = _workspace(dev, "attn", _lib.load().sgf_gram_workspace_bytes(n, m, k))
        with torch.cuda.device(dev):
            _lib.call("sgf_gram_ln_bwd", _ptr(g), _ld(g), _ptr(xin), _ld(xin), _ptr(mean), _ptr(rstd), _ptr(gamma), _ptr(beta),
                      int(relu), m, _ptr(b), _ld(b), k, n, _code(xin), _ptr(out), out.stride(0), _ptr(cs), _ptr(dg), _ptr(db),
                      _ptr(ws), ws.numel(), _stream(dev))
        return out, cs, dg, db

    @staticmethod
    def gram_bn_bwd_supported(m: int, k: int, dtype) -> bool:
        return dtype == _BF16 and bool(_lib.load().sgf_gram_bn_bwd_supported(int(m), int(k), _lib.SGF_BF16))

    @staticmethod
    def gram_bn_bwd(gy, gy2, z, mean, rstd, gamma, beta, relu: bool, stats, inv_n: float, training: bool, b):
        n, m = z.shape
        k = b.shape[1]
        dev = z.device
        out = torch.empty((m, k), dtype=_F32, device=dev)
        cs = torch.empty(m, dtype=_F32, device=dev)
        ws = _workspace(dev, "attn", _lib.load().sgf_gram_workspace_bytes(n, m, k))
        with torch.cuda.device(dev):
            _lib.call("sgf_gram_bn_bwd", _ptr(gy), _ld(gy), _ptr(gy2), _ld(gy2), _ptr(z), _ld(z), _ptr(mean), _ptr(rstd),
                      _ptr(gamma), _ptr(beta), int(relu), _ptr(stats), float(inv_n), int(training), m, _ptr(b), _ld(b), k, n,
                      _code(z), _ptr(out), out.stride(0), _ptr(cs), _ptr(ws), ws.numel(), _stream(dev))
        return out, cs

    @staticmethod
    def gram2_bn_bwd_supported(g, z, b1, b2) -> bool:
        n, m = z.shape
        ok = all(t.dtype == _BF16 and t.dim() == 2 and t.stride(1) == 1 and t.stride(0) % 8 == 0 and t.data_ptr() % 16 == 0
                 for t in (g, z, b1, b2))
        return (ok and b1.shape == b2.shape and g.shape == z.shape
                and bool(_lib.load().sgf_gram2_bn_bwd_supported(int(m), int(b1.shape[1]), int(n), _lib.SGF_BF16)))

    @staticmethod
    def gram2_bn_bwd(g, z, mean, rstd, gamma, beta, relu: bool, stats, inv_n: float, training: bool, b1, b2, out1, out2):
# ... 430 lines not shown
```

### sgformer_amd/linear.py

```python
from __future__ import annotations

import ctypes
from collections import OrderedDict
from typing import Optional

import torch

from . import _lib
from .kernels import (HipKernels, LONG_ROW, _SEGMENT, _code, _ld, _one_pass_cat, _pair_gram, _ptr, _rows,
                      _rows16, _stream, _workspace, _workspaces)

_F32 = torch.float32
_BF16 = torch.bfloat16

from .graph import K


_BN_SAMPLE_ROWS = 1024


def batch_stats(x: torch.Tensor, shard=None):
    K.check(x)
    x = _rows(x.detach())
    n, d = x.shape
# ... 257 lines not shown
    import os
    return (hasattr(K, "gram_ln_bwd_supported") and K.gram_ln_bwd_supported(w1.shape[0], x.shape[1], x.dtype)
            and not x.requires_grad and os.environ.get("SGF_STEM_LN_FUSED", "1") != "0")


def stem_pair_supported(x, w0, w1) -> bool:
    return (x.dim() == 2 and x.shape[0] > 0 and w0.shape == w1.shape and x.stride(-1) == 1
            and (x.stride(0) * x.element_size()) % 8 == 0 and x.data_ptr() % 8 == 0
            and K.stem_pair_supported(x.shape[1], w0.shape[0], x.dtype))


def stem_pair(x, w0, b0, w1, b1, want_stats0=False, shard=None):
    req = {"shard": shard, "out": None} if want_stats0 else None
    y0, y1 = _StemPair.apply(x, w0, b0, w1, b1, req)
    return (y0, y1), (req["out"] if req is not None else None)


def _streaming_linear_ok(x: torch.Tensor, wc: torch.Tensor, dx: bool = False) -> bool:
    return (x.dim() == 2 and x.shape[0] > 0 and wc.stride(-1) == 1 and (wc.stride(0) * wc.element_size()) % 16 == 0
            and wc.data_ptr() % 16 == 0 and x.shape[1] == (wc.shape[0] if dx else wc.shape[1])
            and K.gcn_epilogue_supported(wc.shape[1], wc.shape[0], x.dtype))


def _streaming_linear(xr, wc, b32, shift=None, want_stats=False, rows=None):
    xs = xr if rows is None else [x[:rows] for x in xr]
    if len(xs) == 1:
        return K.gcn_epilogue_stats(xs[0], wc, b32, shift, want_stats=want_stats)
    return K.gcn_epilogue_cat(xs[0], xs[1], wc, b32, shift, want_stats=want_stats)


def _linear_with_stats(xr, wc, b32, stats_req):
    shard = stats_req.get("shard")
    n, d = xr[0].shape[0], wc.shape[0]
    ns = min(n, _BN_SAMPLE_ROWS)
    _, st_s = _streaming_linear(xr, wc, b32, None, want_stats=True, rows=ns)
    n_tot = float(n)
    if shard is None:
        shift = st_s[:d] * (1.0 / float(max(ns, 1)))
    else:
        samp = torch.cat([st_s[:d], torch.full((1,), float(ns), dtype=_F32, device=xr[0].device)])
        shard.all_reduce(samp)
        n_tot = float(shard.n_global)
        shift = (samp[:d] / samp[d].clamp_min(1.0)).contiguous()
    y, st = _streaming_linear(xr, wc, b32, shift, want_stats=True)
    if shard is not None:
        shard.all_reduce(st)
    if stats_req.get("raw"):
        stats_req["out"] = ("raw", st, shift, n_tot)
        return y
    m1 = st[:d] / max(n_tot, 1.0)
    stats_req["out"] = (shift + m1, (st[d:] / max(n_tot, 1.0) - m1 * m1).clamp_min_(0.0), n_tot)
    return y


class GradChain:

    def __init__(self):
        self.acc = None
        self.parts = []


def _fused_bwd() -> bool:
    import os
    return os.environ.get("SGF_GCN_BWD_FUSED", "0") == "1"


def _acc_in_place(d: int, dtype) -> bool:
    import os
    return (hasattr(K, "gcn_epilogue_dx2_acc_supported") and K.gcn_epilogue_dx2_acc_supported(d, dtype)
            and os.environ.get("SGF_GCN_DX_ACC", "1") != "0")


def gcn_layer_fused_ok(x0: torch.Tensor, w: torch.Tensor) -> bool:
    import os
    d = x0.shape[1] if x0.dim() == 2 else 0
    return (x0.dim() == 2 and x0.shape[0] > 0 and x0.dtype == _BF16 and tuple(w.shape) == (d, 2 * d)
            and hasattr(K, "gcn_bn_bwd_dx_supported") and K.gcn_bn_bwd_dx_supported(d, x0.dtype)
            and os.environ.get("SGF_GCN_FUSED", "1") != "0")


class _LinearBNActRes(torch.autograd.Function):

    @staticmethod
    def forward(ctx, y, x0, w, b, gamma, beta, bn_hook, relu: bool, use_res: bool, shard, chain, first: bool):
        K.check(y, x0)
        dt = x0.dtype
        wc = w.detach().to(dt).contiguous()
        b32 = None if b is None else b.detach().float().contiguous()
        yr, xr = _rows16(y), _rows16(x0)
        want = bn_hook(None)
        if want:
            req = {"shard": shard, "out": None, "raw": hasattr(K, "bn_finalize")}
            z = _linear_with_stats([yr, xr], wc, b32, req)
            mean, rstd, n_tot, training = bn_hook(req["out"])
        else:
            z, _ = _streaming_linear([yr, xr], wc, b32)
            mean, rstd, n_tot, training = bn_hook(False)
        g32 = gamma.detach().float().contiguous() if gamma is not None else None
        be32 = beta.detach().float().contiguous() if beta is not None else None
        mean = mean.detach().float().contiguous()
        rstd = rstd.detach().float().contiguous()
        out = K.bn_apply(z, mean, rstd, g32, be32, xr if use_res else None, relu)
        ctx.save_for_backward(yr, xr, z, wc, g32, be32, mean, rstd)
        ctx.meta = (bool(relu), bool(use_res), bool(training), float(n_tot), shard, chain, bool(first), w.dtype,
                    None if b is None else b.dtype, None if gamma is None else gamma.dtype)
        return out

    @staticmethod
    def backward(ctx, gout):
        yr, xr, z, wc, g32, be32, mean, rstd = ctx.saved_tensors
        relu, use_res, training, n_tot, shard, chain, first, wdt, bdt, gdt = ctx.meta
        d = z.shape[1]
        gout = _rows16(gout.contiguous())
        stats = K.bn_bwd_stats(gout, z, mean, rstd, g32, be32, relu)
        if shard is not None:
            shard.all_reduce(stats)
        inv_n = 1.0 / max(n_tot, 1.0)
        if _fused_bwd():
            dz, dy, acc = K.gcn_bn_bwd_dx(gout, z, mean, rstd, g32, be32, relu, stats, inv_n, training, wc, chain.acc,
                                          last=first, add_gy=use_res)
            chain.acc = None if first else acc
            dx0 = acc if first else None
        else:
            fused_dw = None
            if (ctx.needs_input_grad[2] and hasattr(K, "gram2_bn_bwd_supported") and _pair_gram()
                    and K.gram2_bn_bwd_supported(gout, z, yr, xr)):
                dwf = torch.empty((d, 2 * d), dtype=_F32, device=z.device)
                dz, dbf = K.gram2_bn_bwd(gout, z, mean, rstd, g32, be32, relu, stats, inv_n, training, yr, xr, dwf[:, :d], dwf[:, d:])
                fused_dw = (dwf.to(wdt), dbf.to(bdt) if (ctx.needs_input_grad[3] and bdt is not None) else None)
            else:
                dz = K.bn_bwd_apply(gout, z, mean, rstd, g32, be32, relu, stats, inv_n, training)
            if _acc_in_place(d, dz.dtype) and not chain.parts:
                dy, chain.acc = K.gcn_epilogue_dx2_acc(dz, wc, _rows16(gout) if use_res else None, chain.acc)
                dx0 = None
                if first:
                    dx0, chain.acc = chain.acc, None
            else:
                dy, dxi = K.gcn_epilogue_dx2(dz, wc[:, :d], wc[:, d:], True)
                chain.parts.append(dxi)
                if use_res:
                    chain.parts.append(gout)
                dx0 = None
                if first:
                    parts, chain.parts = chain.parts, []
                    if chain.acc is not None:
                        parts.append(chain.acc)
                        chain.acc = None
                    dx0 = parts[0] if len(parts) == 1 else (K.sum_n(parts) if len(parts) <= 8 else sum(parts[1:], parts[0]))
        if not _fused_bwd() and fused_dw is not None:
            dw, db = fused_dw
        else:
            dw, db = _linear_param_grads(dz, [yr, xr], [d, d], ctx.needs_input_grad[2],
                                         ctx.needs_input_grad[3] and bdt is not None, wdt, bdt)
        dgamma = stats[d:].to(gdt) if g32 is not None else None
        dbeta = stats[:d].to(gdt) if be32 is not None else None
        if shard is not None and g32 is not None:
            dgamma, dbeta = shard.unsum(dgamma), shard.unsum(dbeta)
        return dy, dx0, dw, db, dgamma, dbeta, None, None, None, None, None, None


def linear_bn_act_res(y, x0, w, b, gamma, beta, bn_hook, relu, use_res, shard, chain, first):
    return _LinearBNActRes.apply(y, x0, w, b, gamma, beta, bn_hook, relu, use_res, shard, chain, first)


def linear(x, w, b):
    return _Linear.apply(w, b, None, x)


def linear_bn_stats(xs, w, b, shard=None):
    req = {"shard": shard, "out": None}
    xs = xs if isinstance(xs, (tuple, list)) else (xs,)
    y = _Linear.apply(w, b, req, *xs)
    return y, req["out"]


def linear_cat(xs, w, b):
    return _Linear.apply(w, b, None, *xs)


def out_linear_cat(xs, w, b):
    m = w.shape[0]
    if (xs[0].dtype == _F32 and xs[0].is_cuda and m % 4 != 0
            and all(K.gcn_epilogue_supported(x.shape[1], (m + 3) // 4 * 4, _F32) for x in xs)):
        pad = (m + 3) // 4 * 4 - m
        wp = torch.nn.functional.pad(w, (0, 0, 0, pad))
        bp = None if b is None else torch.nn.functional.pad(b, (0, pad))
        return _Linear.apply(wp, bp, None, *xs)[:, :m]
    return _Linear.apply(w, b, None, *xs)


def out_linear(x, w, b):
    m = w.shape[0]
    if (x.dtype == _F32 and x.is_cuda and x.dim() == 2 and m % 4 != 0
            and K.gcn_epilogue_supported(w.shape[1], (m + 3) // 4 * 4, _F32)):
        pad = (m + 3) // 4 * 4 - m
        wp = torch.nn.functional.pad(w, (0, 0, 0, pad))
        bp = None if b is None else torch.nn.functional.pad(b, (0, pad))
        return _Linear.apply(wp, bp, None, x)[:, :m]
    if x.dtype == _BF16 and x.dim() == 2 and m % 8 != 0 and not K.gcn_epilogue_supported(w.shape[1], m, _BF16):
        pad = (m + 7) // 8 * 8 - m
        wp = torch.nn.functional.pad(w, (0, 0, 0, pad))
        bp = None if b is None else torch.nn.functional.pad(b, (0, pad))
        return _Linear.apply(wp, bp, None, x)[:, :m]
    return _Linear.apply(w, b, None, x)
```

### sgformer_amd/ours.py

```python
from __future__ import annotations

import torch
import torch.nn as nn
import torch.nn.functional as F

from . import ops

__all__ = ["GraphConvLayer", "GraphConv", "TransConvLayer", "TransConv", "SGFormer",
           "full_attention_conv"]

_NO_SHARD = None

DEFAULT_COMPUTE_DTYPE = None

import os as _os
OVERLAP_BRANCHES = _os.environ.get("SGF_OVERLAP", "1") == "1"
OVERLAP_MIN_NODES = 65536
_side_streams = {}


def _side_stream(device):
    s = _side_streams.get(device.index)
    if s is None:
        s = _side_streams[device.index] = torch.cuda.Stream(device=device)
    return s


class _Holder:
    _x_cache = None


import weakref as _weakref
_entry_cache = _weakref.WeakKeyDictionary()


def _stem_w(lin: nn.Linear, x):
    f = lin.weight.shape[1]
    pad = x.shape[1] - f
    if pad != 0 and x.shape[1] not in ((f + 3) // 4 * 4, (f + 7) // 8 * 8):
        raise RuntimeError(f"input has {x.shape[1]} features, the layer expects {f}")
    return lin.weight if pad == 0 else F.pad(lin.weight, (0, pad))


def _entry_width(f: int, cdt) -> int:
    q = 8 if cdt == torch.bfloat16 else 4
    return (f + q - 1) // q * q


def _lin(x, lin: nn.Linear):
    return ops.linear(x, _stem_w(lin, x), lin.bias)


def _drop(x, p, training, res=None):
    if training and p is not None and p > 0.0:
        if x.dim() == 2 and x.shape[1] % 4 == 0:
            return ops.dropout_res(x, res, float(p))
        x = F.dropout(x, p=p, training=True)
        return x if res is None else x + res
    if p is None:
        raise TypeError("dropout probability is None (pass --trans_dropout / --gnn_dropout)")
    return x if res is None else x + res


def full_attention_conv(qs, ks, vs, output_attn=False, shard=None):
    n, h, d = qs.shape
    qk = torch.cat([qs.reshape(n, h * d), ks.reshape(n, h * d)], dim=1)
    if vs.shape[1] == h:
        qkv = torch.cat([qk, vs.reshape(n, h * d)], dim=1)
        out = ops.attention(qkv, None, h, d, shard, per_head=h > 1)
    else:
        out = ops.attention(qk, vs.reshape(n, d), h, d, shard, per_head=h > 1)
    out = out.reshape(n, h, d)
    if output_attn:
        return out, _attention_matrix(qs, ks)
    return out


def _attention_matrix(qs, ks):
    n = qs.shape[0]
    qn = qs / torch.norm(qs, p=2)
    kn = ks / torch.norm(ks, p=2)
    attention = torch.einsum("nhm,lhm->nlh", qn, kn).mean(dim=-1)
    normalizer = (torch.einsum("nhm,hm->nh", qn, kn.sum(dim=0)) + n).mean(dim=-1, keepdim=True)
    return attention / normalizer


def _uses_batch_stats(module: nn.Module, bn: nn.BatchNorm1d) -> bool:
    return module.training or not bn.track_running_stats or bn.running_mean is None


class GraphConvLayer(nn.Module):

    def __init__(self, in_channels, out_channels, use_weight=True, use_init=False):
        super().__init__()
        self.use_init = use_init
        self.use_weight = use_weight
        in_channels_ = 2 * in_channels if use_init else in_channels
        self.W = nn.Linear(in_channels_, out_channels)
        self._shard = _NO_SHARD

    def reset_parameters(self):
        self.W.reset_parameters()

    def propagate(self, x, edge_index):
        shard = self._shard
        if isinstance(edge_index, ops.CSRGraph):
            graph = edge_index
        elif shard is not None and not shard.local_graph:
            graph = shard.graph_for(edge_index)
        else:
            graph = ops.graph_cache.get(edge_index, x.shape[0])
        return ops.spmm(graph, x, None if (shard is not None and shard.local_graph) else shard)

    def forward(self, x, edge_index, x0, bn_stats=False):
        shard = self._shard
        y = self.propagate(x, edge_index)
        if self.use_init:
            if bn_stats:
                return ops.linear_bn_stats((y, x0), self.W.weight, self.W.bias, shard)
            y = ops.linear_cat((y, x0), self.W.weight, self.W.bias)
        elif self.use_weight:
            if bn_stats:
                return ops.linear_bn_stats(y, self.W.weight, self.W.bias, shard)
            y = _lin(y, self.W)
        return (y, None) if bn_stats else y


class GraphConv(nn.Module):

    def __init__(self, in_channels, hidden_channels, num_layers=2, dropout=0.5, use_bn=True,
                 use_residual=True, use_weight=True, use_init=False, use_act=True):
        super().__init__()
        self.convs = nn.ModuleList()
        self.fcs = nn.ModuleList()
        self.fcs.append(nn.Linear(in_channels, hidden_channels))
        self.bns = nn.ModuleList()
        self.bns.append(nn.BatchNorm1d(hidden_channels))
        for _ in range(num_layers):
            self.convs.append(GraphConvLayer(hidden_channels, hidden_channels, use_weight, use_init))
            self.bns.append(nn.BatchNorm1d(hidden_channels))
        self.dropout = dropout
        self.activation = F.relu
        self.use_bn = use_bn
        self.use_residual = use_residual
        self.use_act = use_act
        self._shard = _NO_SHARD

    def reset_parameters(self):
        for conv in self.convs:
            conv.reset_parameters()
        for bn in self.bns:
            bn.reset_parameters()
        for fc in self.fcs:
            fc.reset_parameters()

    def _bn_act_res(self, bn: nn.BatchNorm1d, x, res, relu, stats=None):
        shard = self._shard
        use_batch = _uses_batch_stats(self, bn)
        if use_batch:
            mean, var, n_tot = stats if stats is not None else ops.batch_stats(x, shard)
            if n_tot <= 1 and self.training:
                raise ValueError("Expected more than 1 value per channel when training")
            if self.training and bn.track_running_stats and bn.running_mean is not None:
                with torch.no_grad():
                    bn.num_batches_tracked += 1
                    m = bn.momentum if bn.momentum is not None else 1.0 / float(bn.num_batches_tracked)
                    bn.running_mean.mul_(1.0 - m).add_(mean.to(bn.running_mean.dtype), alpha=m)
                    unbiased = var * (n_tot / max(n_tot - 1.0, 1.0))
                    bn.running_var.mul_(1.0 - m).add_(unbiased.to(bn.running_var.dtype), alpha=m)
        else:
            mean, var, n_tot = bn.running_mean.float(), bn.running_var.float(), float(x.shape[0])
        rstd = torch.rsqrt(var + bn.eps)
        return ops.bn_act_res(x, res, bn.weight, bn.bias, mean, rstd, relu, use_batch, n_tot, shard)

    def _bn_hook(self, bn: nn.BatchNorm1d):
        def hook(stats):
            use_batch = _uses_batch_stats(self, bn)
            if stats is None:
                return use_batch
            if use_batch and stats[0] == "raw":
                _, sums, shift, n_tot = stats
                if n_tot <= 1 and self.training:
                    raise ValueError("Expected more than 1 value per channel when training")
                track = self.training and bn.track_running_stats and bn.running_mean is not None
                if track and bn.momentum is not None and bn.running_mean.dtype == torch.float32:
                    with torch.no_grad():
                        bn.num_batches_tracked += 1
                        mean, rstd = ops.K.bn_finalize(sums, shift, n_tot, bn.eps, float(bn.momentum), bn.running_mean,
                                                       bn.running_var)
                    return mean, rstd, n_tot, True
                if not track:
                    mean, rstd = ops.K.bn_finalize(sums, shift, n_tot, bn.eps, 0.0, None, None)
                    return mean, rstd, n_tot, True
                d = sums.numel() // 2
                m1 = sums[:d] / max(n_tot, 1.0)
                stats = ((shift + m1) if shift is not None else m1, (sums[d:] / max(n_tot, 1.0) - m1 * m1).clamp_min_(0.0),
                         n_tot)
            if use_batch:
                mean, var, n_tot = stats
                if n_tot <= 1 and self.training:
                    raise ValueError("Expected more than 1 value per channel when training")
                if self.training and bn.track_running_stats and bn.running_mean is not None:
                    with torch.no_grad():
                        bn.num_batches_tracked += 1
                        m = bn.momentum if bn.momentum is not None else 1.0 / float(bn.num_batches_tracked)
                        bn.running_mean.mul_(1.0 - m).add_(mean.to(bn.running_mean.dtype), alpha=m)
                        unbiased = var * (n_tot / max(n_tot - 1.0, 1.0))
                        bn.running_var.mul_(1.0 - m).add_(unbiased.to(bn.running_var.dtype), alpha=m)
            else:
                mean, var, n_tot = bn.running_mean.float(), bn.running_var.float(), 0.0
            return mean, torch.rsqrt(var + bn.eps), n_tot, use_batch
        return hook

    def fused_stem_ok(self, x) -> bool:
        import os
        d = self.fcs[0].out_features
        drop_on = self.training and self.dropout is not None and self.dropout > 0.0
        return (self.use_bn and not drop_on and len(self.convs) > 0 and all(c.use_init for c in self.convs)
                and x.dim() == 2 and x.dtype == torch.bfloat16
                and all(tuple(c.W.weight.shape) == (d, 2 * d) for c in self.convs)
                and hasattr(ops.K, "gcn_bn_bwd_dx_supported") and ops.K.gcn_bn_bwd_dx_supported(d, x.dtype)
                and os.environ.get("SGF_GCN_FUSED", "1") != "0" and os.environ.get("SGF_STEM_FUSED", "1") != "0")

    def _fused_layers(self, x0):
        drop_on = self.training and self.dropout is not None and self.dropout > 0.0
        return (self.use_bn and not drop_on and len(self.convs) > 0 and all(c.use_init for c in self.convs)
                and all(ops.gcn_layer_fused_ok(x0, c.W.weight) for c in self.convs))

    def _stage(self, bn, x, res, relu, stats=None):
        drop_on = self.training and self.dropout is not None and self.dropout > 0.0
        fuse_res = res is not None and not drop_on
        if self.use_bn:
            x = self._bn_act_res(bn, x, res if fuse_res else None, relu, stats)
        else:
            if relu:
                x = torch.relu(x)
            if fuse_res:
                x = x + res
        return _drop(x, self.dropout, self.training, res if (res is not None and not fuse_res) else None)

    def forward(self, x, edge_index, stem=None):
        ops._require_cuda(x, None if isinstance(edge_index, ops.CSRGraph) else edge_index)
        x_first = None
        if stem is not None and len(stem) == 3:
            _, x, x_first = stem
        else:
            if stem is not None:
                x, stats0 = stem
            else:
                x, stats0 = _lin(x, self.fcs[0]), None
            x = self._stage(self.bns[0], x, None, True, stats0)
        if self._fused_layers(x):
            x0, chain = x, ops.GradChain()
            if x_first is not None:
                x = x_first
            for i, conv in enumerate(self.convs):
                bn = self.bns[i + 1]
                y = conv.propagate(x, edge_index)
                x = ops.linear_bn_act_res(y, x0, conv.W.weight, conv.W.bias, bn.weight, bn.bias, self._bn_hook(bn),
                                          self.use_act, self.use_residual, self._shard, chain, i == 0)
            return x
        uses_init = [c.use_init for c in self.convs]
        k = 1 + sum(uses_init) + (len(self.convs) if self.use_residual else 0)
        hub = list(ops.fan_out(x, k)) if k <= 8 else [x] * k
        x = hub.pop()
        for i, conv in enumerate(self.convs):
            want = self.use_bn and _uses_batch_stats(self, self.bns[i + 1])
            x0 = hub.pop() if uses_init[i] else None
            if want:
                x, stats = conv(x, edge_index, x0, bn_stats=True)
            else:
                x, stats = conv(x, edge_index, x0), None
            x = self._stage(self.bns[i + 1], x, hub.pop() if self.use_residual else None, self.use_act, stats)
        return x


class TransConvLayer(nn.Module):

    def __init__(self, in_channels, out_channels, num_heads, use_weight=True):
        super().__init__()
        self.Wk = nn.Linear(in_channels, out_channels * num_heads)
        self.Wq = nn.Linear(in_channels, out_channels * num_heads)
        if use_weight:
            self.Wv = nn.Linear(in_channels, out_channels * num_heads)
        self.out_channels = out_channels
        self.num_heads = num_heads
        self.use_weight = use_weight
        self._shard = _NO_SHARD

    def reset_parameters(self):
        self.Wk.reset_parameters()
        self.Wq.reset_parameters()
        if self.use_weight:
            self.Wv.reset_parameters()

    def _project(self, query_input, source_input):
        ws = [self.Wq.weight, self.Wk.weight] + ([self.Wv.weight] if self.use_weight else [])
        bs = [self.Wq.bias, self.Wk.bias] + ([self.Wv.bias] if self.use_weight else [])
        if query_input is source_input:
            return ops.linear(query_input, torch.cat(ws, 0), torch.cat(bs, 0))
        q = ops.linear(query_input, ws[0], bs[0])
        kv = ops.linear(source_input, torch.cat(ws[1:], 0), torch.cat(bs[1:], 0))
        return torch.cat([q, kv], 1)

    def forward(self, query_input, source_input, output_attn=False, grad_tap=None):
        ops._require_cuda(query_input, source_input)
        h, d = self.num_heads, self.out_channels
        if (h == 1 and query_input is source_input and not output_attn and query_input.shape[1] == d
                and d % 4 == 0 and d <= 256):
            wv, bv = (self.Wv.weight, self.Wv.bias) if self.use_weight else (None, None)
            return ops.attention_from_input(query_input, self.Wq.weight, self.Wq.bias, self.Wk.weight,
                                            self.Wk.bias, wv, bv, self._shard, tap=grad_tap)
        qkv = self._project(query_input, source_input)
        v_ext = None
        if not self.use_weight:
            if source_input.shape[1] != d:
                raise RuntimeError(f"use_weight=False needs in_channels == out_channels ({d})")
            v_ext = source_input
        final_output = ops.attention(qkv, v_ext, h, d, self._shard)
        if output_attn:
            n = qkv.shape[0]
            qs = qkv[:, :h * d].reshape(n, h, d)
            ks = qkv[:, h * d:2 * h * d].reshape(n, h, d)
            return final_output, _attention_matrix(qs, ks)
        return final_output


class TransConv(nn.Module):

    def __init__(self, in_channels, hidden_channels, num_layers=2, num_heads=1, dropout=0.5,
                 use_bn=True, use_residual=True, use_weight=True, use_act=True, alpha=None,
                 layer_cls=None):
        super().__init__()
        layer_cls = layer_cls or TransConvLayer
        self.convs = nn.ModuleList()
        self.fcs = nn.ModuleList()
        self.fcs.append(nn.Linear(in_channels, hidden_channels))
        self.bns = nn.ModuleList()
        self.bns.append(nn.LayerNorm(hidden_channels))
        for _ in range(num_layers):
            self.convs.append(layer_cls(hidden_channels, hidden_channels, num_heads=num_heads,
                                        use_weight=use_weight))
            self.bns.append(nn.LayerNorm(hidden_channels))
# ... 236 lines not shown
```

Baseline: 29.37 million.

## Fuse BN scale-shift, ReLU and residual into the next GCN layer's SpMM gather

In the fused GCN layer chain, the BatchNorm apply, ReLU and residual add are no longer materialised between layers. The BN statistics are folded into per-channel scale and shift. The next SpMM applies relu(scale*z+shift) to each gathered neighbour row and adds the first layer's propagated output as the precomputed A·x0 residual term. This removes one full elementwise pass per layer, meaning a write and a re-read of an n×d activation. In exchange it adds per-edge FMA and max work, and it forces the plain row kernel instead of the heuristically chosen SpMM variant. The path is restricted to bf16, 128<d<=256, unsharded graphs without long rows, and can be disabled with an env flag.

```diff
diff --git a/include/sgf.h b/include/sgf.h
--- a/include/sgf.h
+++ b/include/sgf.h
@@ -8,7 +8,7 @@
 extern "C" {
 #endif
 
-#define SGF_VERSION 661
+#define SGF_VERSION 662
 
 #define SGF_F32 0
 #define SGF_BF16 1
@@ -62,6 +62,11 @@
 int sgf_spmm(const int64_t* rowptr, const int32_t* colind, const float* val, const void* x,
              int64_t ldx, int64_t n_cols, void* y, int64_t ldy, int64_t n_rows, int32_t d,
              int32_t dtype, void* stream);
+
+int32_t sgf_spmm_bnact_supported(int32_t d, int32_t dtype);
+int sgf_spmm_bnact(const int64_t* rowptr, const int32_t* colind, const float* val, const void* z, int64_t ldz,
+                   int64_t n_cols, const float* scale, const float* shift, const void* y_add, int64_t ldadd, void* y,
+                   int64_t ldy, int64_t n_rows, int32_t d, int32_t dtype, void* stream);
 
 int32_t sgf_spmm_segment_len(void);
 size_t sgf_spmm_split_workspace_bytes(int64_t long_segments, int32_t d);
@@ -245,6 +250,8 @@
                  void* stream);
 int sgf_bn_finalize(const float* sums, const float* shift, double n_total, float eps, float momentum, float* running_mean,
                     float* running_var, int32_t d, float* mean, float* rstd, void* stream);
+int sgf_bn_scale_shift(const float* mean, const float* rstd, const float* gamma, const float* beta, int32_t d, float* scale,
+                       float* shift, void* stream);
 int sgf_bn_apply(const void* x, int64_t ldx, const float* mean, const float* rstd,
                  const float* gamma, const float* beta, const void* res, int64_t ldr,
                  int32_t relu, int64_t n, int32_t d, int32_t dtype, void* y, int64_t ldy,
diff --git a/sgformer_amd/_lib.py b/sgformer_amd/_lib.py
--- a/sgformer_amd/_lib.py
+++ b/sgformer_amd/_lib.py
@@ -37,6 +37,9 @@
     "sgf_graph_prologue_plan": (c_int32, [_P, c_int64, c_int64, c_int32, c_int32, c_int32, _P, _P, c_size_t, _P]),
     "sgf_graph_prologue_emit": (c_int32, [c_int64, c_int64, c_int32, c_int32, c_int64, _P, _P, c_size_t, _P]),
     "sgf_spmm": (c_int32, [_P, _P, _P, _P, c_int64, c_int64, _P, c_int64, c_int64, c_int32, c_int32, _P]),
+    "sgf_spmm_bnact_supported": (c_int32, [c_int32, c_int32]),
+    "sgf_spmm_bnact": (c_int32, [_P, _P, _P, _P, c_int64, c_int64, _P, _P, _P, c_int64, _P, c_int64, c_int64, c_int32, c_int32,
+                                 _P]),
     "sgf_spmm_segment_len": (c_int32, []),
     "sgf_spmm_split_workspace_bytes": (c_size_t, [c_int64, c_int32]),
     "sgf_spmm_split": (c_int32, [_P, _P, _P, _P, c_int64, c_int64, _P, c_int64, c_int64, c_int32, c_int32, c_int64,
@@ -132,6 +135,7 @@
     "sgf_colstats_workspace_bytes": (c_size_t, [c_int64, c_int32]),
     "sgf_colstats": (c_int32, [_P, c_int64, _P, c_int64, c_int32, c_int32, _P, _P, c_size_t, _P]),
     "sgf_bn_finalize": (c_int32, [_P, _P, c_double, c_float, c_float, _P, _P, c_int32, _P, _P, _P]),
+    "sgf_bn_scale_shift": (c_int32, [_P, _P, _P, _P, c_int32, _P, _P, _P]),
     "sgf_bn_apply": (c_int32, [_P, c_int64, _P, _P, _P, _P, _P, c_int64, c_int32, c_int64, c_int32,
                                c_int32, _P, c_int64, _P]),
     "sgf_bn_bwd_stats": (c_int32, [_P, c_int64, _P, c_int64, _P, _P, _P, _P, c_int32, c_int64, c_int32,
diff --git a/sgformer_amd/csrc/fused.hip b/sgformer_amd/csrc/fused.hip
--- a/sgformer_amd/csrc/fused.hip
+++ b/sgformer_amd/csrc/fused.hip
@@ -1415,6 +1415,26 @@
   const float unbias = static_cast<float>(n_total / (n_total - 1.0 > 1.0 ? n_total - 1.0 : 1.0));
   hipLaunchKernelGGL(k_bn_finalize, dim3((d + 255) / 256), dim3(256), 0, static_cast<hipStream_t>(stream), sums, shift,
                      static_cast<float>(1.0 / nn), unbias, eps, momentum, running_mean, running_var, d, mean, rstd);
+  SGF_LAUNCH_CHECK();
+  return SGF_OK;
+}
+
+__global__ __launch_bounds__(256) void k_bn_scale_shift(const float* __restrict__ mean, const float* __restrict__ rstd,
+                                                        const float* __restrict__ gamma, const float* __restrict__ beta,
+                                                        int d, float* __restrict__ scale, float* __restrict__ shift) {
+  const int c = blockIdx.x * 256 + threadIdx.x;
+  if (c >= d) return;
+  const float a = rstd[c] * (gamma ? gamma[c] : 1.f);
+  scale[c] = a;
+  shift[c] = fmaf(-mean[c], a, beta ? beta[c] : 0.f);
+}
+
+extern "C" int sgf_bn_scale_shift(const float* mean, const float* rstd, const float* gamma, const float* beta, int32_t d,
+                                  float* scale, float* shift, void* stream) {
+  SGF_REQUIRE(d >= 1, SGF_E_INVALID, "sgf_bn_scale_shift: bad size");
+  SGF_REQUIRE(mean && rstd && scale && shift, SGF_E_INVALID, "sgf_bn_scale_shift: null pointer");
+  hipLaunchKernelGGL(k_bn_scale_shift, dim3((d + 255) / 256), dim3(256), 0, static_cast<hipStream_t>(stream), mean, rstd,
+                     gamma, beta, d, scale, shift);
   SGF_LAUNCH_CHECK();
   return SGF_OK;
 }
diff --git a/sgformer_amd/csrc/spmm.hip b/sgformer_amd/csrc/spmm.hip
--- a/sgformer_amd/csrc/spmm.hip
+++ b/sgformer_amd/csrc/spmm.hip
@@ -89,10 +89,33 @@
   }
 };
 
-template <typename T, int N>
+struct BnActArgs {
+  const float* scale;
+  const float* shift;
+  const void* y_add;
+  int64_t ldadd;
+};
+template <bool XF> struct RowXf;
+template <> struct RowXf<false> {
+  __device__ __forceinline__ void load(const BnActArgs&, int, bool) {}
+  __device__ __forceinline__ float4 operator()(const float4& z) const { return z; }
+};
+template <> struct RowXf<true> {
+  float4 a, b;
+  __device__ __forceinline__ void load(const BnActArgs& p, int col, bool active) {
+    a = active ? *reinterpret_cast<const float4*>(p.scale + col) : make_float4(0.f, 0.f, 0.f, 0.f);
+    b = active ? *reinterpret_cast<const float4*>(p.shift + col) : make_float4(0.f, 0.f, 0.f, 0.f);
+  }
+  __device__ __forceinline__ float4 operator()(const float4& z) const {
+    return make_float4(fmaxf(fmaf(a.x, z.x, b.x), 0.f), fmaxf(fmaf(a.y, z.y, b.y), 0.f),
+                       fmaxf(fmaf(a.z, z.z, b.z), 0.f), fmaxf(fmaf(a.w, z.w, b.w), 0.f));
+  }
+};
+
+template <typename T, int N, bool XF>
 __device__ __forceinline__ void gather_batch(__amdgpu_buffer_rsrc_t rsrc, int voff, uint32_t pitch,
                                              const int32_t* __restrict__ colind, const float* __restrict__ val,
-                                             int e, float4& acc) {
+                                             int e, float4& acc, const RowXf<XF>& xf) {
   int32_t c[N];
   float v[N];
   typename BufRow<T>::Raw raw[N];
@@ -104,14 +127,14 @@
 #pragma unroll
   for (int u = 0; u < N; ++u) raw[u] = BufRow<T>::load(rsrc, voff, static_cast<uint32_t>(c[u]) * pitch);
 #pragma unroll
-  for (int u = 0; u < N; ++u) fma4(acc, v[u], BufRow<T>::widen(raw[u]));
-}
-
-template <typename T, int UNROLL>
+  for (int u = 0; u < N; ++u) fma4(acc, v[u], xf(BufRow<T>::widen(raw[u])));
+}
+
+template <typename T, int UNROLL, bool XF = false>
 __global__ __launch_bounds__(kWavesPerBlock * 64) void k_spmm_row(
     const int64_t* __restrict__ rowptr, const int32_t* __restrict__ colind, const float* __restrict__ val,
     const T* __restrict__ x, uint32_t pitch, uint32_t x_bytes, T* __restrict__ y, int64_t ldy, int64_t n_rows,
-    int32_t d, LongQueue lq) {
+    int32_t d, LongQueue lq, BnActArgs xa) {
   const int lane = threadIdx.x & 63;
   const int wid = __builtin_amdgcn_readfirstlane(static_cast<int>(threadIdx.x >> 6));
   const int64_t blk = xcd_remap(blockIdx.x, gridDim.x);
@@ -128,6 +151,10 @@
   const bool active = fc < d;
   const int voff = active ? fc * static_cast<int>(sizeof(T)) : 0;
   float4 acc = make_float4(0.f, 0.f, 0.f, 0.f);
+  RowXf<XF> xf;
+  xf.load(xa, fc, active);
+  float4 add = make_float4(0.f, 0.f, 0.f, 0.f);
+  if (XF && active) add = load4<T>(static_cast<const T*>(xa.y_add) + row * xa.ldadd + fc);
   const int32_t* __restrict__ ci = colind + e0;
   const float* __restrict__ va = val + e0;
   const int len = static_cast<int>(e1 - e0);
@@ -154,7 +181,7 @@
         }
       }
 #pragma unroll
-      for (int u = 0; u < UNROLL; ++u) fma4(acc, v0[u], BufRow<T>::widen(raw[u]));
+      for (int u = 0; u < UNROLL; ++u) fma4(acc, v0[u], xf(BufRow<T>::widen(raw[u])));
       if (!more_a) break;
 #pragma unroll
       for (int u = 0; u < UNROLL; ++u) raw[u] = BufRow<T>::load(rsrc, voff, static_cast<uint32_t>(c1[u]) * pitch);
@@ -168,13 +195,14 @@
         }
       }
 #pragma unroll
-      for (int u = 0; u < UNROLL; ++u) fma4(acc, v1[u], BufRow<T>::widen(raw[u]));
+      for (int u = 0; u < UNROLL; ++u) fma4(acc, v1[u], xf(BufRow<T>::widen(raw[u])));
       if (!more_b) break;
     }
   }
-  if (i + 4 <= len) { gather_batch<T, 4>(rsrc, voff, pitch, ci, va, i, acc); i += 4; }
-  if (i + 2 <= len) { gather_batch<T, 2>(rsrc, voff, pitch, ci, va, i, acc); i += 2; }
-  if (i < len) gather_batch<T, 1>(rsrc, voff, pitch, ci, va, i, acc);
+  if (i + 4 <= len) { gather_batch<T, 4, XF>(rsrc, voff, pitch, ci, va, i, acc, xf); i += 4; }
+  if (i + 2 <= len) { gather_batch<T, 2, XF>(rsrc, voff, pitch, ci, va, i, acc, xf); i += 2; }
+  if (i < len) gather_batch<T, 1, XF>(rsrc, voff, pitch, ci, va, i, acc, xf);
+  if (XF) { acc.x += add.x; acc.y += add.y; acc.z += add.z; acc.w += add.w; }
   if (active) store4<T>(y + row * ldy + fc, acc);
 }
 
@@ -982,6 +1010,7 @@
 enum Forced { kForceNone = -1, kForceWave, kForceRow, kForceSeg, kForceSeg2, kForceSub };
 const char* const kForcedWords[] = {"wave", "row", "seg", "seg2", "sub"};
 EnvWord g_forced{"SGF_SPMM_KERNEL", kForcedWords, 5};
+EnvInt g_bnact{"SGF_SPMM_BNACT", 1};
 
 template <typename T>
 int launch_blocked(const int64_t* rowptr, const int32_t* ecode, const float* eval, const int32_t* nlds,
@@ -1055,7 +1084,7 @@
 template <typename T>
 int launch(const int64_t* rowptr, const int32_t* colind, const float* val, const T* x, int64_t ldx, int64_t n_cols,
            T* y, int64_t ldy, int64_t n_rows, int32_t d, hipStream_t st, const LongQueue& lq,
-           float* partial, bool stream) {
+           float* partial, bool stream, const BnActArgs* xf = nullptr) {
   constexpr int UNROLL = 8;
   const dim3 block(kWavesPerBlock * 64);
   const uint64_t x_bytes = static_cast<uint64_t>(n_cols) * static_cast<uint64_t>(ldx) * sizeof(T);
@@ -1064,6 +1093,18 @@
                        reinterpret_cast<uintptr_t>(y) % 16 == 0;
   const Choice c = choose_kernel(d, sizeof(T), fits32, pair_ok, stream, g_forced.get());
   const int64_t nb = (n_rows + kWavesPerBlock - 1) / kWavesPerBlock;
+  if (xf != nullptr) {
+    if constexpr (sizeof(T) == 2) {
+      SGF_REQUIRE(fits32 && d > 128, SGF_E_UNSUPPORTED,
+                  "sgf_spmm_bnact: 128 < d <= 256 and n_cols * ldz * 2 < 2^32 (the row kernel's 32-bit offsets)");
+      hipLaunchKernelGGL((k_spmm_row<T, UNROLL, true>), dim3(static_cast<unsigned>(nb)), block, 0, st, rowptr, colind, val,
+                         x, static_cast<uint32_t>(ldx * sizeof(T)), static_cast<uint32_t>(x_bytes), y, ldy, n_rows, d, lq,
+                         *xf);
+      SGF_LAUNCH_CHECK();
+      return SGF_OK;
+    }
+    SGF_REQUIRE(false, SGF_E_UNSUPPORTED, "sgf_spmm_bnact: bf16 storage only");
+  }
   const int64_t nbs = (n_rows + kWavesPerBlock * kSegRows - 1) / (kWavesPerBlock * kSegRows);
   const int chunk_rows = g_chunk_rows.get() > 0 ? g_chunk_rows.get() : 4096;
   const int chunk = chunk_rows / (kWavesPerBlock * kSegRows) > 0 ? chunk_rows / (kWavesPerBlock * kSegRows) : 1;
@@ -1088,7 +1129,7 @@
     case Arm::Row:
       hipLaunchKernelGGL((k_spmm_row<T, UNROLL>), dim3(static_cast<unsigned>(nb)), block, 0, st, rowptr, colind,
                          val, x, static_cast<uint32_t>(ldx * sizeof(T)), static_cast<uint32_t>(x_bytes), y, ldy,
-                         n_rows, d, lq);
+                         n_rows, d, lq, BnActArgs{nullptr, nullptr, nullptr, 0});
       break;
     case Arm::Wave:
       hipLaunchKernelGGL((k_spmm_wave<T, UNROLL>), dim3(static_cast<unsigned>(nb)), block, 0, st,
@@ -1152,7 +1193,7 @@
 
 int spmm_common(const int64_t* rowptr, const int32_t* colind, const float* val, const void* x, int64_t ldx,
                 int64_t n_cols, void* y, int64_t ldy, int64_t n_rows, int32_t d, int32_t dtype, const LongQueue& lq,
-                float* partial, hipStream_t st, const char* fn, bool stream = false) {
+                float* partial, hipStream_t st, const char* fn, bool stream = false, const BnActArgs* xf = nullptr) {
   SGF_REQUIRE(n_rows >= 0 && d >= 0 && n_cols >= 0, SGF_E_INVALID, "%s: negative size", fn);
   if (n_rows == 0 || d == 0) return SGF_OK;
   SGF_REQUIRE(rowptr && x && y, SGF_E_INVALID, "%s: null pointer", fn);
@@ -1161,9 +1202,9 @@
   if (const int rc = check_spmm_operands(fn, x, ldx, y, ldy, d, dtype)) return rc;
   if (dtype == SGF_F32)
     return launch<float>(rowptr, colind, val, static_cast<const float*>(x), ldx, n_cols, static_cast<float*>(y), ldy,
-                         n_rows, d, st, lq, partial, stream);
+                         n_rows, d, st, lq, partial, stream, xf);
   return launch<uint16_t>(rowptr, colind, val, static_cast<const uint16_t*>(x), ldx, n_cols,
-                          static_cast<uint16_t*>(y), ldy, n_rows, d, st, lq, partial, stream);
+                          static_cast<uint16_t*>(y), ldy, n_rows, d, st, lq, partial, stream, xf);
 }
 }
 
@@ -1173,6 +1214,29 @@
   const LongQueue none{nullptr, nullptr, 0, INT64_MAX};
   return spmm_common(rowptr, colind, val, x, ldx, n_cols, y, ldy, n_rows, d, dtype, none, nullptr,
                      static_cast<hipStream_t>(stream), "sgf_spmm");
+}
+
+extern "C" int32_t sgf_spmm_bnact_supported(int32_t d, int32_t dtype) {
+  return dtype == SGF_BF16 && d % 4 == 0 && d > 128 && d <= 256 && g_bnact.get() != 0;
+}
+
+extern "C" int sgf_spmm_bnact(const int64_t* rowptr, const int32_t* colind, const float* val, const void* z, int64_t ldz,
+                              int64_t n_cols, const float* scale, const float* shift, const void* y_add, int64_t ldadd,
+                              void* y, int64_t ldy, int64_t n_rows, int32_t d, int32_t dtype, void* stream) {
+  const char* fn = "sgf_spmm_bnact";
+  SGF_REQUIRE(dtype == SGF_BF16, SGF_E_UNSUPPORTED, "%s: bf16 storage only (dtype %d)", fn, dtype);
+  SGF_REQUIRE(d >= 0 && d <= 256 && (d == 0 || d > 128), SGF_E_UNSUPPORTED, "%s: d = %d outside (128, 256]", fn, d);
+  if (n_rows > 0 && d > 0) {
+    SGF_REQUIRE(scale && shift && y_add, SGF_E_INVALID, "%s: null pointer", fn);
+    SGF_REQUIRE(reinterpret_cast<uintptr_t>(scale) % 16 == 0 && reinterpret_cast<uintptr_t>(shift) % 16 == 0, SGF_E_INVALID,
+                "%s: scale / shift must be 16-byte aligned", fn);
+    SGF_REQUIRE(ldadd % 4 == 0 && ldadd >= d && reinterpret_cast<uintptr_t>(y_add) % 8 == 0, SGF_E_INVALID,
+                "%s: y_add must be aligned to 4 elements, ldadd a multiple of 4 with ldadd >= d", fn);
+  }
+  const LongQueue none{nullptr, nullptr, 0, INT64_MAX};
+  const BnActArgs xf{scale, shift, y_add, ldadd};
+  return spmm_common(rowptr, colind, val, z, ldz, n_cols, y, ldy, n_rows, d, dtype, none, nullptr,
+                     static_cast<hipStream_t>(stream), fn, false, &xf);
 }
 
 extern "C" int32_t sgf_spmm_segment_len(void) { return kSegLen; }
diff --git a/sgformer_amd/graph.py b/sgformer_amd/graph.py
--- a/sgformer_amd/graph.py
+++ b/sgformer_amd/graph.py
@@ -77,6 +77,17 @@
             self._t = (self.rowptr, self.colind, self.val) if sym else (t_rowptr, t_colind, t_val)
             self.t_long_segments = self.long_segments if sym else long_row_segments(t_rowptr, self.nnz)
         return self._t
+
+    def has_long_rows(self) -> bool:
+        if self.long_segments == 0:
+            return False
+        exact = getattr(self, "_has_long_rows", None)
+        if exact is None:
+            if torch.cuda.is_available() and torch.cuda.is_current_stream_capturing():
+                return True
+            lens = self.rowptr[1:] - self.rowptr[:-1]
+            exact = self._has_long_rows = bool(int(lens.max()) > LONG_ROW) if lens.numel() > 0 else False
+        return exact
 
     blocked = False
     _t_lazy = False
@@ -407,5 +418,29 @@
     return K.spmm(rp, ci, va, x, graph.n, out=out, long_segments=segs)
 
 
+class _SpMMBnAct(torch.autograd.Function):
+
+    @staticmethod
+    def forward(ctx, z, graph, scale, shift, y_add):
+        K.check(z, y_add)
+        ctx.graph = graph
+        return K.spmm_bnact(graph.rowptr, graph.colind, graph.val, z, scale, shift, y_add, graph.n)
+
+    @staticmethod
+    def backward(ctx, gy):
+        return spmm_on(ctx.graph, gy.contiguous(), True), None, None, None, None
+
+
+def spmm_bnact_ok(graph, x: torch.Tensor) -> bool:
+    return (hasattr(K, "spmm_bnact_supported") and x.dim() == 2 and K.spmm_bnact_supported(x.shape[1], x.dtype)
+            and not graph.has_long_rows() and graph.n == x.shape[0]
+            and not (getattr(graph, "blocked", False) or getattr(graph, "tiled", False) or getattr(graph, "locality", False))
+            and x.shape[0] * x.shape[1] * x.element_size() < 2 ** 32)
+
+
+def spmm_bnact(graph, z: torch.Tensor, scale, shift, y_add: torch.Tensor) -> torch.Tensor:
+    return _SpMMBnAct.apply(z, graph, scale, shift, y_add.detach())
+
+
 def spmm(graph, x: torch.Tensor, shard=None) -> torch.Tensor:
     return _SpMM.apply(x, graph, shard)
diff --git a/sgformer_amd/graphed.py b/sgformer_amd/graphed.py
--- a/sgformer_amd/graphed.py
+++ b/sgformer_amd/graphed.py
@@ -86,6 +86,9 @@
         self.long_segments = self.t_long_segments = int(long_segments)
         self.symmetric = True
         self._t = (self.rowptr, self.colind, self.val)
+
+    def has_long_rows(self) -> bool:
+        return self.long_segments > 0
 
     def load(self, rowptr, colind, val):
         nnz = self.nnz = int(colind.numel())
diff --git a/sgformer_amd/kernels.py b/sgformer_amd/kernels.py
--- a/sgformer_amd/kernels.py
+++ b/sgformer_amd/kernels.py
@@ -304,6 +304,24 @@
         return y
 
     @staticmethod
+    def spmm_bnact_supported(d: int, dtype) -> bool:
+        return dtype == _BF16 and bool(_lib.load().sgf_spmm_bnact_supported(int(d), _lib.SGF_BF16))
+
+    @staticmethod
+    def spmm_bnact(rowptr, colind, val, z: torch.Tensor, scale, shift, y_add: torch.Tensor, n_rows: int) -> torch.Tensor:
+        z, y_add = _rows(z), _rows(y_add)
+        d = z.shape[1]
+        if y_add.shape != (n_rows, d) or y_add.dtype != z.dtype:
+            raise ValueError("spmm_bnact: y_add must be [n_rows, d] in the storage dtype of z")
+        y = torch.empty((n_rows, d), dtype=z.dtype, device=z.device)
+        if n_rows == 0 or d == 0:
+            return y
+        with torch.cuda.device(z.device):
+            _lib.call("sgf_spmm_bnact", _ptr(rowptr), _ptr(colind), _ptr(val), _ptr(z), z.stride(0), z.shape[0], _ptr(scale),
+                      _ptr(shift), _ptr(y_add), y_add.stride(0), _ptr(y), y.stride(0), n_rows, d, _code(z), _stream(z.device))
+        return y
+
+    @staticmethod
     def reorder(ei: torch.Tensor, n: int, iters1: int, iters2: int):
         dev, nnz = ei.device, int(ei.shape[1])
         perm = torch.empty(n, dtype=torch.int32, device=dev)
@@ -713,6 +731,16 @@
             _lib.call("sgf_bn_finalize", _ptr(sums), _ptr(shift), float(n_total), float(eps), float(momentum),
                       _ptr(running_mean), _ptr(running_var), d, _ptr(mean), _ptr(rstd), _stream(sums.device))
         return mean, rstd
+
+    @staticmethod
+    def bn_scale_shift(mean, rstd, gamma, beta):
+        d = mean.numel()
+        scale = torch.empty(d, dtype=_F32, device=mean.device)
+        shift = torch.empty(d, dtype=_F32, device=mean.device)
+        with torch.cuda.device(mean.device):
+            _lib.call("sgf_bn_scale_shift", _ptr(mean), _ptr(rstd), _ptr(gamma), _ptr(beta), d, _ptr(scale), _ptr(shift),
+                      _stream(mean.device))
+        return scale, shift
 
     @staticmethod
     def bn_apply(x, mean, rstd, gamma, beta, res, relu: bool) -> torch.Tensor:
diff --git a/sgformer_amd/linear.py b/sgformer_amd/linear.py
--- a/sgformer_amd/linear.py
+++ b/sgformer_amd/linear.py
@@ -363,7 +363,7 @@
 class _LinearBNActRes(torch.autograd.Function):
 
     @staticmethod
-    def forward(ctx, y, x0, w, b, gamma, beta, bn_hook, relu: bool, use_res: bool, shard, chain, first: bool):
+    def forward(ctx, y, x0, w, b, gamma, beta, bn_hook, relu: bool, use_res: bool, shard, chain, first: bool, defer=None):
         K.check(y, x0)
         dt = x0.dtype
         wc = w.detach().to(dt).contiguous()
@@ -381,7 +381,11 @@
         be32 = beta.detach().float().contiguous() if beta is not None else None
         mean = mean.detach().float().contiguous()
         rstd = rstd.detach().float().contiguous()
-        out = K.bn_apply(z, mean, rstd, g32, be32, xr if use_res else None, relu)
+        if defer is not None:
+            defer["scale"], defer["shift"] = K.bn_scale_shift(mean, rstd, g32, be32)
+            out = z
+        else:
+            out = K.bn_apply(z, mean, rstd, g32, be32, xr if use_res else None, relu)
         ctx.save_for_backward(yr, xr, z, wc, g32, be32, mean, rstd)
         ctx.meta = (bool(relu), bool(use_res), bool(training), float(n_tot), shard, chain, bool(first), w.dtype,
                     None if b is None else b.dtype, None if gamma is None else gamma.dtype)
@@ -437,11 +441,11 @@
         dbeta = stats[:d].to(gdt) if be32 is not None else None
         if shard is not None and g32 is not None:
             dgamma, dbeta = shard.unsum(dgamma), shard.unsum(dbeta)
-        return dy, dx0, dw, db, dgamma, dbeta, None, None, None, None, None, None
-
-
-def linear_bn_act_res(y, x0, w, b, gamma, beta, bn_hook, relu, use_res, shard, chain, first):
-    return _LinearBNActRes.apply(y, x0, w, b, gamma, beta, bn_hook, relu, use_res, shard, chain, first)
+        return dy, dx0, dw, db, dgamma, dbeta, None, None, None, None, None, None, None
+
+
+def linear_bn_act_res(y, x0, w, b, gamma, beta, bn_hook, relu, use_res, shard, chain, first, defer=None):
+    return _LinearBNActRes.apply(y, x0, w, b, gamma, beta, bn_hook, relu, use_res, shard, chain, first, defer)
 
 
 def linear(x, w, b):
diff --git a/sgformer_amd/ours.py b/sgformer_amd/ours.py
--- a/sgformer_amd/ours.py
+++ b/sgformer_amd/ours.py
@@ -102,15 +102,17 @@
     def reset_parameters(self):
         self.W.reset_parameters()
 
+    def graph_of(self, x, edge_index):
+        shard = self._shard
+        if isinstance(edge_index, ops.CSRGraph):
+            return edge_index
+        if shard is not None and not shard.local_graph:
+            return shard.graph_for(edge_index)
+        return ops.graph_cache.get(edge_index, x.shape[0])
+
     def propagate(self, x, edge_index):
         shard = self._shard
-        if isinstance(edge_index, ops.CSRGraph):
-            graph = edge_index
-        elif shard is not None and not shard.local_graph:
-            graph = shard.graph_for(edge_index)
-        else:
-            graph = ops.graph_cache.get(edge_index, x.shape[0])
-        return ops.spmm(graph, x, None if (shard is not None and shard.local_graph) else shard)
+        return ops.spmm(self.graph_of(x, edge_index), x, None if (shard is not None and shard.local_graph) else shard)
 
     def forward(self, x, edge_index, x0, bn_stats=False):
         shard = self._shard
@@ -227,6 +229,13 @@
         return (self.use_bn and not drop_on and len(self.convs) > 0 and all(c.use_init for c in self.convs)
                 and all(ops.gcn_layer_fused_ok(x0, c.W.weight) for c in self.convs))
 
+    def _bnact_graph(self, x0, edge_index):
+        if not (self._shard is None and all(c._shard is None for c in self.convs) and self.use_act and self.use_residual
+                and len(self.convs) > 1):
+            return None
+        graph = self.convs[0].graph_of(x0, edge_index)
+        return graph if ops.spmm_bnact_ok(graph, x0) else None
+
     def _stage(self, bn, x, res, relu, stats=None):
         drop_on = self.training and self.dropout is not None and self.dropout > 0.0
         fuse_res = res is not None and not drop_on
@@ -254,11 +263,19 @@
             x0, chain = x, ops.GradChain()
             if x_first is not None:
                 x = x_first
+            graph = self._bnact_graph(x0, edge_index)
+            y1 = handoff = None
             for i, conv in enumerate(self.convs):
                 bn = self.bns[i + 1]
-                y = conv.propagate(x, edge_index)
+                if handoff is not None:
+                    y = ops.spmm_bnact(graph, x, handoff["scale"], handoff["shift"], y1)
+                else:
+                    y = conv.propagate(x, edge_index)
+                if i == 0:
+                    y1 = y
+                handoff = {} if (graph is not None and i + 1 < len(self.convs)) else None
                 x = ops.linear_bn_act_res(y, x0, conv.W.weight, conv.W.bias, bn.weight, bn.bias, self._bn_hook(bn),
-                                          self.use_act, self.use_residual, self._shard, chain, i == 0)
+                                          self.use_act, self.use_residual, self._shard, chain, i == 0, handoff)
             return x
         uses_init = [c.use_init for c in self.convs]
         k = 1 + sum(uses_init) + (len(self.convs) if self.use_residual else 0)
```

Result: no change. 29.60 million (median of 6 runs) (+0.8%).
